# seongeunryu/lime-cikm25

Hardware: AMD Instinct MI355X
Metric: impressions scored/sec (higher is better)
Workload: dtype f32

## Files before the change

include/lime_hip.h:

```cpp
#ifndef LIME_HIP_H
#define LIME_HIP_H

#include <stdint.h>

#ifdef __cplusplus
extern "C" {
#endif

#define LIME_ABI_VERSION 14

typedef enum {
    LIME_OK = 0,
    LIME_ERR_BAD_ARG = -1,
    LIME_ERR_UNSUPPORTED = -2,
    LIME_ERR_LAUNCH = -3,
    LIME_NOT_APPLICABLE = 1
} lime_status;

int lime_abi_version(void);
const char* lime_last_error_string(void);
int64_t lime_device_cus(void);

enum { LIME_ACT_NONE = 0, LIME_ACT_RELU = 1, LIME_ACT_TANH = 2, LIME_ACT_SIGMOID = 3,
       LIME_ACT_RELU_GRAD = 4  };
// ... 97 lines not shown

int64_t lime_ffn_pack_sp_size(int32_t F, int32_t which);
int lime_ffn_pack_sp(const float* w1, int64_t ldw1, const float* w2, int64_t ldw2, int32_t E, int32_t F, uint16_t* w1p, uint16_t* w2p,
                     void* stream);

typedef struct {
    const float* attn;    int64_t lda;
    const uint16_t* wp;
    const float* bias;
    const float* res;     int64_t ldr;
    const int32_t* res_ids;
    const float* res_pe;  int64_t ldr_pe;
    int32_t res_period;
    float ln_eps;
    const float* ln_gamma; const float* ln_beta;
    float* out;           int64_t ldo;
    int32_t M, E;
    const int32_t* m_dev;
} lime_oproj_sp_args;

int lime_encoder_oproj_sp(const lime_oproj_sp_args* args, void* stream);

int64_t lime_oproj_pack_sp_size(void);
int lime_oproj_pack_sp(const float* w, int64_t ldw, int32_t E, uint16_t* wp, void* stream);

typedef struct {
    const uint16_t* attn; int64_t lda;
    const uint16_t* w0p;
    const float* add_rows; int64_t ld_add; int32_t add_period;
    int32_t res_kind;
    const uint16_t* res;  int64_t ldr;  int64_t res_rows;
    const int32_t* res_ids;
    const float* ln1_gamma; const float* ln1_beta; float ln1_eps;
    int32_t pool32;
    const uint16_t* w1p;  const uint16_t* w2p;  const float* b2;
    const float* ln2_gamma; const float* ln2_beta; float ln2_eps;
    int32_t M, E, F;
    void* out;            int64_t ldo;
    const int32_t* m_dev;
} lime_encoder_block_bf16_args;

int lime_encoder_block_bf16(const lime_encoder_block_bf16_args* args, void* stream);

int64_t lime_oproj_pack_bf16_size(void);
int lime_oproj_pack_bf16(const float* w, int64_t ldw, int32_t E, uint16_t* wp, void* stream);

typedef struct {
    const uint16_t* a;   int64_t lda;  int64_t a_rows;  const int32_t* a_ids;
    const uint16_t* wp;
    const float* add_rows; int64_t ld_add; int32_t add_period;
    int32_t M, N, K;
    int32_t reserved;
    const int32_t* c_ids;
    uint16_t* out;       int64_t ldo;  int64_t out_rows;
    const int32_t* m_dev;
} lime_inproj_bf16_args;

int lime_inproj_bf16(const lime_inproj_bf16_args* args, void* stream);
int64_t lime_inproj_pack_bf16_size(int32_t N);
int lime_inproj_pack_bf16(const float* w, int64_t ldw, int32_t N, int32_t K, uint16_t* wp, void* stream);

int32_t lime_ffn_bf16_model_columns(void);

int lime_to_bf16(const float* src, int64_t lds, int64_t rows, int32_t cols, uint16_t* dst, int64_t ldd, int64_t rows_out,
                 int32_t cols_out, void* stream);

int lime_mean_pool_bf16(const uint16_t* x, int64_t ldx, float* out, int64_t ldo, int32_t n_seq, int32_t S, int32_t dim,
                        void* stream);

int lime_embed_pe_f32(const int32_t* ids, const float* table, int64_t ld_table, const float* pe, int64_t ld_pe,
                      int32_t period, float* out, int64_t ldo, int64_t rows, int32_t dim, void* stream);

int lime_compact_sequences(const int32_t* ids, int32_t n_seq, int32_t S, int32_t pad_base, int32_t* seq_inv, int32_t* ids_c,
                           int32_t* row_map, int32_t* tok_ids, int32_t* tok_rows, int32_t* counts, int32_t* work, void* stream);

int lime_fill_pad_rows_f32(const int32_t* ids, const float* src, int64_t lds, float* dst, int64_t ldd, int64_t rows, int32_t S, int32_t cols,
                           void* stream);
int64_t lime_compact_sequences_workspace(int32_t n_seq);

int lime_compact_batch(const int32_t* ids_t, int32_t T, int32_t pad_base_t, int32_t* seq_inv_t, int32_t* ids_c_t, int32_t* row_map_t,
                       int32_t* tok_ids_t, int32_t* tok_rows_t, int32_t* counts_t, const int32_t* ids_b, int32_t L, int32_t pad_base_b,
                       int32_t* seq_inv_b, int32_t* ids_c_b, int32_t* row_map_b, int32_t* tok_ids_b, int32_t* tok_rows_b, int32_t* counts_b,
                       int32_t n, const int32_t* cat, const int32_t* sub, const float* fresh, const float* life, int32_t count_mult,
                       int32_t* news_src, int32_t* news_inv, int32_t* title_row, int32_t* body_row, int32_t* cat_c, int32_t* sub_c,
                       float* fresh_c, float* life_c, int32_t* news_counts, int32_t* work, void* stream);
int64_t lime_compact_batch_workspace(int32_t n);

int lime_news_xin_f32(const float* title_blocks, int64_t ld_t, int32_t nblk_t, const float* body_blocks, int64_t ld_b, int32_t nblk_b,
                      const int32_t* title_row, const int32_t* body_row, const int32_t* n_news, float* xin, int64_t ldx, int32_t cap,
                      int32_t dim, void* stream);

enum { LIME_ATTN_FORM_PLAIN = 0, LIME_ATTN_FORM_COUNT = 1, LIME_ATTN_FORM_LSE = 2, LIME_ATTN_FORM_ROWS = 3, LIME_ATTN_FORM_VOCAB = 4,
       LIME_ATTN_FORM_DROPOUT = 5 };
typedef struct {
    const float* q;
    const float* k;
    const float* v;
    int64_t ld_qkv;
    const float* pos_rows;
    const int32_t* row_map;
    const uint8_t* key_mask;
    const int32_t* n_seq_dev;
    float* lse;
    float* out;
    int64_t ldo;
    float* workspace;
    int64_t workspace_floats;
    uint64_t dropout_seed;
    float dropout_p;
    uint32_t dropout_site;
    int32_t n_seq, S, n_head, head_dim, head_stride;
    float scale;
    int32_t form;
    int32_t reserved;
} lime_token_attention_args;

int lime_token_attention_f32(const lime_token_attention_args* args, void* stream);

enum { LIME_ATTN_NONE = 0, LIME_ATTN_SP = 1, LIME_ATTN_SP_LONG = 2, LIME_ATTN_SP_VOCAB = 3, LIME_ATTN_MFMA = 4, LIME_ATTN_WIDE = 5,
       LIME_ATTN_DROPOUT = 6, LIME_ATTN_DROPOUT_LONG = 7 };
enum { LIME_ATTN_STATS_NONE = 0, LIME_ATTN_STATS_FP32 = 1, LIME_ATTN_STATS_SPLIT = 2 };
typedef struct {
    int32_t family;
    int32_t stats_pass;
    int32_t n_launches;
    int32_t reserved;
    char name[2][64];
} lime_token_attention_plan;

int lime_token_attention_plan_f32(const lime_token_attention_args* args, lime_token_attention_plan* out);

int lime_token_attention_rows_bf16(const uint16_t* q, const uint16_t* k, const uint16_t* v, int64_t ld_qkv, const int32_t* row_map,
                                   const int32_t* n_seq_dev, uint16_t* out, int64_t ldo, int32_t n_seq, int32_t S, int32_t n_head,
                                   int32_t head_dim, float scale, int32_t out_cols, void* stream);

int lime_token_attention_bf16(const uint16_t* q, const uint16_t* k, const uint16_t* v, int64_t ld_qkv, uint16_t* out,
                              int64_t ldo, int32_t n_seq, int32_t S, int32_t n_head, int32_t head_dim, float scale,
                              int32_t out_cols, void* stream);

int lime_pad_heads_f32(const float* src, int64_t lds, float* dst, int64_t ldd, int32_t n_blk, int32_t head_dim,
                       int32_t head_stride, int32_t cols, void* stream);

int lime_mean_pool_f32(const float* x, int64_t ldx, float* out, int64_t ldo, int32_t n_seq, int32_t S, int32_t dim,
                       void* stream);
int lime_mean_pool_count_f32(const float* x, int64_t ldx, float* out, int64_t ldo, int32_t n_seq, int32_t S, int32_t dim,
                             const int32_t* n_seq_dev, void* stream);

int lime_bucketize_f32(const float* x, int32_t* out, int64_t n, void* stream);
int lime_bucketize_cuts_f32(const float* x, const float* cuts, int32_t n_cuts, int32_t* out, int64_t n, void* stream);

int lime_topic_rep_f32(const int32_t* cat, const int32_t* sub, const float* cat_table, const float* sub_table,
                       int32_t dc, int32_t ds, const float* w, const float* bias, int32_t dout, float* out, int64_t ldo,
                       float* emb_out, int64_t ld_emb, int64_t rows, void* stream);

int lime_intent_fuse_f32(const float* intents, const float* att_hidden, const float* affine2_t, const float* affine2_b,
                         float* content, int64_t ldc, int64_t M, int32_t k, int32_t D, int32_t A, void* stream);
int lime_intent_fuse_count_f32(const float* intents, const float* att_hidden, const float* affine2_t, const float* affine2_b,
                               float* content, int64_t ldc, int64_t M, int32_t k, int32_t D, int32_t A, const int32_t* m_dev, void* stream);

int lime_additive_pool_f32(const float* hidden, int64_t ldh, const float* affine2, int32_t A, const float* x, int64_t ldx,
                           int32_t D, const uint8_t* mask, float* out, int64_t ldo, int32_t n_seq, int32_t S, void* stream);
int lime_additive_pool_count_f32(const float* hidden, int64_t ldh, const float* affine2, int32_t A, const float* x, int64_t ldx, int32_t D,
                                 const uint8_t* mask, const int32_t* n_seq_dev, float* out, int64_t ldo, int32_t n_seq, int32_t S, void* stream);

int lime_cand_attn_weights_f32(const float* qp, const float* kp, const uint8_t* mask, float* agg, int32_t B, int32_t N,
                               int32_t H, int32_t D, int32_t n_head, void* stream);
int64_t lime_cand_attn_weights_workspace(int32_t B, int32_t N, int32_t H, int32_t n_head);
int lime_cand_attn_weights_ws_f32(const float* qp, const float* kp, const uint8_t* mask, float* agg, int32_t B, int32_t N, int32_t H,
                                  int32_t D, int32_t n_head, float* workspace, int64_t workspace_floats, void* stream);
int lime_cand_attn_weights_shared_f32(const float* qp, const float* kp, const uint8_t* mask, float* agg, int32_t B, int32_t N, int32_t H,
                                      int32_t D, int32_t n_head, int32_t hist_div, float* workspace, int64_t workspace_floats, void* stream);

int lime_gate_ln_f32(const float* y, const float* x, const float* scale, const float* bias, const float* gamma,
                     const float* beta, float eps, float* out, int64_t rows, int32_t D, void* stream);

int lime_gate_ln_sage_f32(const float* y, const float* x, const float* scale, const float* bias, const float* gamma, const float* beta,
                          float eps, float* out, const float* node_const, float* mean_out, int64_t groups, int32_t H, int32_t D,
                          int32_t row_div, int32_t n_src, void* stream);

int lime_sage_mean_f32(const float* hist, const float* user_nodes, float* out, int32_t B, int32_t H, int32_t n_user,
                       int32_t n_src, int32_t D, void* stream);

int lime_interest_match_f32(const float* kp, const float* qp, const float* g, const float* cand, const float* remaining,
                            float* user_rep, float* logits, int32_t B, int32_t N, int32_t H, int32_t A, int32_t D,
                            float scale, float alpha_s, float beta_s, int32_t use_weight, int32_t use_penalty,
                            void* stream);

int lime_lifetime_score_f32(const float* user, const float* news, const float* remaining, float* logits, int64_t rows,
                            int32_t D, float alpha_s, float beta_s, int32_t use_weight, int32_t use_penalty, void* stream);

int lime_row_scale_f32(const float* x, const float* scale, float* out, int64_t rows, int32_t D, void* stream);

int lime_mhsa_live_ids(const int32_t* ids, const uint8_t* mask, int32_t n_seq, int32_t T, int32_t* ids_eff, void* stream);
int lime_mhsa_compact_mask(int32_t* ids_c, const int32_t* seq_src, const uint8_t* mask, int32_t n_compact_slots, int32_t T,
                           uint8_t* mask_c, void* stream);

int lime_fuse_rows_f32(const float* a, int64_t lda, const float* b, int64_t ldb, const float* gate, int64_t ldg, float* out, int64_t ldo,
                       int64_t rows, int32_t cols, void* stream);

int lime_gather_rows_f32(const int32_t* idx, const float* table, int64_t ld_table, float* out, int64_t ldo, int64_t rows,
                         int32_t dim, void* stream);

#define LIME_MAX_COPIES 32
typedef struct {
    const void* src;
    void* dst;
    int64_t bytes;
} lime_copy_desc;
int lime_multi_copy(const lime_copy_desc* descs, int32_t n, void* stream);

#define LIME_MAX_GATHERS 16
typedef struct {
    const void* table;  int64_t table_stride;
    void* out;          int64_t out_stride;
    int32_t row_bytes;  int32_t reserved;
} lime_gather_desc;
int lime_gather_rows_multi(const int32_t* idx, int64_t n_rows, const lime_gather_desc* descs, int32_t n, void* stream);


int64_t lime_linear_wgrad_workspace(int32_t M, int32_t N, int32_t K);
int lime_linear_wgrad_f32(const float* dy, int64_t ldy, const float* x, int64_t ldx, float* dw, int64_t lddw, float* db,
                          int32_t M, int32_t N, int32_t K, int32_t accumulate, float* workspace, int64_t workspace_floats,
                          void* stream);

int64_t lime_colsum_workspace(int32_t M, int32_t N);
int lime_colsum_f32(const float* x, int64_t ldx, int32_t M, int32_t N, float* out, int32_t accumulate, float* workspace,
                    int64_t workspace_floats, void* stream);

int64_t lime_layernorm_bwd_workspace(int32_t M, int32_t E);
int lime_layernorm_bwd_f32(const float* dy, int64_t lddy, int32_t dy_div, float dy_scale, const float* y, int64_t ldy,
                           const float* gamma, const float* beta, const float* rstd, float* dz, int64_t lddz, int32_t M,
                           int32_t E, float* dgamma, float* dbeta, float* dzsum, int32_t accumulate, float* workspace,
                           int64_t workspace_floats, void* stream);
int lime_layernorm_bwd_dropout_f32(const float* dy, int64_t lddy, int32_t dy_div, float dy_scale, const float* y, int64_t ldy,
                                   const float* gamma, const float* beta, const float* rstd, float* dz, int64_t lddz, int32_t M, int32_t E,
                                   float* dgamma, float* dbeta, float* dzsum, int32_t accumulate, float* workspace,
                                   int64_t workspace_floats, float* dz_drop, int64_t lddd, float dropout_p, uint64_t seed, uint32_t site,
                                   void* stream);

int lime_relu_bwd_f32(float* dh, int64_t lddh, const float* h, int64_t ldh, int64_t rows, int32_t cols, float scale, void* stream);

int64_t lime_token_attention_bwd_workspace(int32_t n_seq, int32_t S, int32_t n_head);
int64_t lime_token_attention_stats_workspace(int32_t n_seq, int32_t S, int32_t n_head);
int64_t lime_token_attention_bwd_workspace_wide(int32_t n_seq, int32_t S, int32_t n_head, int32_t head_dim);
enum { LIME_BWD_ATTN_ENTRY_PLAIN = 0, LIME_BWD_ATTN_ENTRY_LSE = 1 };
typedef struct {
    const float* q;
    const float* k;
    const float* v;
    int64_t ld_qkv;
    const float* out;
    int64_t ld_out;
    const float* lse;
    const float* dout;
    int64_t ldo;
    float* dq;
    float* dk;
    float* dv;
    int64_t ld_dqkv;
    float* workspace;
    int64_t workspace_floats;
    const uint8_t* key_mask;
    uint64_t dropout_seed;
    float dropout_p;
    uint32_t dropout_site;
    int32_t n_seq, S, n_head, head_dim, head_stride;
    float scale;
    int32_t entry;
    int32_t reserved;
} lime_token_attention_bwd_args;

int lime_token_attention_bwd_f32(const lime_token_attention_bwd_args* args, void* stream);

enum { LIME_BWD_ATTN_NONE = 0, LIME_BWD_ATTN_ONE_PASS = 1, LIME_BWD_ATTN_SP = 2, LIME_BWD_ATTN_LONG = 3, LIME_BWD_ATTN_LONG_SP = 4,
       LIME_BWD_ATTN_WIDE = 5 };
enum { LIME_BWD_ATTN_PASS_NONE = 0, LIME_BWD_ATTN_PASS_STATS_FP32 = 1, LIME_BWD_ATTN_PASS_STATS_SPLIT = 2, LIME_BWD_ATTN_PASS_DELTA = 3 };
typedef struct {
    int32_t family;
    int32_t stats_pass;
    int32_t n_launches;
    int32_t reserved;
    char name[3][64];
} lime_token_attention_bwd_plan;

int lime_token_attention_bwd_plan_f32(const lime_token_attention_bwd_args* args, lime_token_attention_bwd_plan* out);

int lime_additive_pool_bwd_f32(const float* hidden, int64_t ldh, const float* affine2, int32_t A, const float* x, int64_t ldx, int32_t D,
                               const uint8_t* mask, const float* dout, int64_t ldo, float* dhidden, int64_t lddh, float* dx, int64_t lddx,
                               float* da2_part, int32_t n_seq, int32_t S, void* stream);


int lime_dropout_f32(const float* src, int64_t lds, float* dst, int64_t ldd, int64_t rows, int32_t cols, float p, uint64_t seed,
                     uint32_t site, void* stream);
int lime_dropout2_f32(const float* src, int64_t lds, float* dst, int64_t ldd, int64_t rows, int32_t cols, float p, uint64_t seed,
                      uint32_t site1, uint32_t site2, void* stream);

int lime_embed_pe_dropout_f32(const int32_t* ids, const float* table, int64_t ld_table, const float* pe, int64_t ld_pe,
                              int32_t period, float* out, int64_t ldo, int64_t rows, int32_t dim, float p, uint64_t seed,
                              uint32_t site_emb, uint32_t site_pe, void* stream);

int lime_dropout_add_layernorm_f32(const float* t, int64_t ldt, const float* res, int64_t ldr, const float* gamma, const float* beta,
                                   float eps, float* y, int64_t ldy, float* rstd, int64_t M, int32_t E, float p, uint64_t seed,
                                   uint32_t site, void* stream);

int lime_embed_bwd_f32(const int32_t* ids, const float* dx, int64_t lddx, float* dtable, int64_t ld_table, int64_t rows,
                       int32_t dim, int32_t hot_id, void* stream);
// ... 222 lines not shown
```

lime_cikm25_amd/csrc/compact.hip:

```cpp
#include "common.h"

namespace {

__device__ __forceinline__ void count_seq(const int* __restrict__ ids, int s, int S, int* __restrict__ live_cnt) {
    const int lane = threadIdx.x & 63;
    int c = 0;
    for (int t = lane; t < S; t += 64) c += ids[(long)s * S + t] != 0;
#pragma unroll
    for (int o = 32; o > 0; o >>= 1) c += __shfl_xor(c, o);
    if (lane == 0) live_cnt[s] = c;
}

__global__ __launch_bounds__(256) void seq_count_kernel(const int* __restrict__ ids, int n_seq, int S, int* __restrict__ live_cnt) {
    const int s = blockIdx.x * 4 + (threadIdx.x >> 6);
    if (s >= n_seq) return;
    count_seq(ids, s, S, live_cnt);
}

__global__ __launch_bounds__(1024) void seq_scan_kernel(const int* __restrict__ live_cnt, int n_seq, int S, int* __restrict__ seq_src,
                                                        int* __restrict__ seq_inv, int* __restrict__ tok_off, int* __restrict__ counts) {
    __shared__ int part_seq[1024], part_tok[1024];
    const int tid = threadIdx.x;
    const int per = (n_seq + 1023) / 1024;
    const int lo = tid * per, hi = min(n_seq, lo + per);
    int ns = 0, nt = 0;
    for (int s = lo; s < hi; ++s) {
        const int c = live_cnt[s];
        ns += c > 0;
        nt += c;
    }
    part_seq[tid] = ns;
    part_tok[tid] = nt;
    __syncthreads();
    for (int o = 1; o < 1024; o <<= 1) {
        int a = 0, b = 0;
        if (tid >= o) { a = part_seq[tid - o]; b = part_tok[tid - o]; }
        __syncthreads();
        part_seq[tid] += a;
        part_tok[tid] += b;
        __syncthreads();
    }
    const int n_live = part_seq[1023], n_tok = part_tok[1023];
    int ps = part_seq[tid] - ns, pt = part_tok[tid] - nt;
    for (int s = lo; s < hi; ++s) {
        const int c = live_cnt[s];
        if (c > 0) {
            seq_src[ps] = s;
            seq_inv[s] = ps;
            tok_off[ps] = pt;
            ++ps;
            pt += c;
        } else {
            seq_inv[s] = n_live;
        }
    }
    for (int i = n_live + 1 + tid; i <= n_seq; i += 1024) seq_src[i] = -1;
    if (tid == 0) {
        seq_src[n_live] = -1;
        tok_off[n_live] = n_tok;
        counts[0] = n_live + 1;
        counts[1] = (n_live + 1) * S;
        counts[2] = n_tok;
        counts[3] = n_live;
        counts[4] = n_tok + S;
    }
}

__device__ __forceinline__ void emit_seq(const int cs, const int* __restrict__ ids, int S, const int* __restrict__ seq_src,
                                         const int* __restrict__ tok_off, const int* __restrict__ counts, int pad_base,
                                         int* __restrict__ ids_c, int* __restrict__ row_map, int* __restrict__ tok_ids,
                                         int* __restrict__ tok_rows) {
    const int lane = threadIdx.x & 63;
    const int n_c = counts[0];
    if (cs >= n_c) return;
    const int src = seq_src[cs];
    int base = tok_off[cs];
    for (int t0 = 0; t0 < S; t0 += 64) {
        const int t = t0 + lane;
        int id = 0;
        if (t < S && src >= 0) id = ids[(long)src * S + t];
        const bool live = id != 0;
        const unsigned long long m = __ballot(live);
        if (t < S) {
            const int row = cs * S + t;
            ids_c[row] = id;
            row_map[row] = live ? row : pad_base + t;
            if (cs == n_c - 1) {
                tok_ids[base + t] = 0;
                tok_rows[base + t] = pad_base + t;
            }
            if (live) {
                const int k = base + __popcll(m & ((1ull << lane) - 1ull));
                tok_ids[k] = id;
                tok_rows[k] = row;
            }
        }
        base += __popcll(m);
    }
}

__global__ __launch_bounds__(256) void seq_emit_kernel(const int* __restrict__ ids, int n_seq, int S, const int* __restrict__ seq_src,
                                                       const int* __restrict__ tok_off, const int* __restrict__ counts, int pad_base,
                                                       int* __restrict__ ids_c, int* __restrict__ row_map, int* __restrict__ tok_ids,
                                                       int* __restrict__ tok_rows) {
    emit_seq(blockIdx.x * 4 + (threadIdx.x >> 6), ids, S, seq_src, tok_off, counts, pad_base, ids_c, row_map, tok_ids, tok_rows);
}

struct SeqSide {
    const int* ids; int S, pad_base;
    int *live_cnt, *seq_src, *tok_off;
    int *seq_inv, *ids_c, *row_map, *tok_ids, *tok_rows, *counts;
};
struct NewsSide {
    const int *cat, *sub, *fresh, *life;
    int *news_src, *news_inv, *title_row, *body_row, *cat_c, *sub_c, *fresh_c, *life_c, *counts;
    int count_mult;
};

__global__ __launch_bounds__(256) void batch_count_kernel(const SeqSide t, const SeqSide b, int n) {
    const int w = blockIdx.x * 4 + (threadIdx.x >> 6);
    if (w >= 2 * n) return;
    if (w < n) count_seq(t.ids, w, t.S, t.live_cnt);
    else count_seq(b.ids, w - n, b.S, b.live_cnt);
}

__device__ __forceinline__ void scan_side_write(const SeqSide& d, int n, int lo, int hi, int ps, int pt, int n_live, int n_tok) {
    const int tid = threadIdx.x;
    for (int s = lo; s < hi; ++s) {
        const int c = d.live_cnt[s];
        if (c > 0) {
            d.seq_src[ps] = s;
            d.seq_inv[s] = ps;
            d.tok_off[ps] = pt;
            ++ps;
            pt += c;
        } else {
            d.seq_inv[s] = n_live;
        }
    }
    for (int i = n_live + 1 + tid; i <= n; i += 1024) d.seq_src[i] = -1;
    if (tid == 0) {
        d.seq_src[n_live] = -1;
        d.tok_off[n_live] = n_tok;
        d.counts[0] = n_live + 1;
        d.counts[1] = (n_live + 1) * d.S;
        d.counts[2] = n_tok;
        d.counts[3] = n_live;
        d.counts[4] = n_tok + d.S;
    }
}

__global__ __launch_bounds__(1024) void batch_scan_kernel(const SeqSide t, const SeqSide b, const NewsSide w, int n) {
    __shared__ int part[5][1024];
    const int tid = threadIdx.x;
    const int per = (n + 1023) / 1024;
    const int lo = min(n, tid * per), hi = min(n, lo + per);
    int first = 0x7FFFFFFF;
    for (int s = hi - 1; s >= lo; --s)
        if (t.live_cnt[s] == 0 && b.live_cnt[s] == 0) first = s;
    part[0][tid] = first;
    __syncthreads();
    for (int o = 512; o > 0; o >>= 1) {
        if (tid < o) part[0][tid] = min(part[0][tid], part[0][tid + o]);
        __syncthreads();
    }
    first = part[0][0];
    __syncthreads();
    const bool has_pad = first != 0x7FFFFFFF;
    int kc = 0, ks = 0, kf = 0, kl = 0;
    if (has_pad) { kc = w.cat[first]; ks = w.sub[first]; kf = w.fresh[first]; kl = w.life[first]; }
    auto repeats = [&](int s) {
        return has_pad && t.live_cnt[s] == 0 && b.live_cnt[s] == 0 && w.cat[s] == kc && w.sub[s] == ks && w.fresh[s] == kf && w.life[s] == kl;
    };
    int v[5] = {0, 0, 0, 0, 0};
    for (int s = lo; s < hi; ++s) {
        const int ct = t.live_cnt[s], cb = b.live_cnt[s];
        v[0] += ct > 0; v[1] += ct;
        v[2] += cb > 0; v[3] += cb;
        v[4] += !repeats(s);
    }
#pragma unroll
    for (int i = 0; i < 5; ++i) part[i][tid] = v[i];
    __syncthreads();
    for (int o = 1; o < 1024; o <<= 1) {
        int a[5] = {0, 0, 0, 0, 0};
        if (tid >= o) {
#pragma unroll
            for (int i = 0; i < 5; ++i) a[i] = part[i][tid - o];
        }
        __syncthreads();
#pragma unroll
        for (int i = 0; i < 5; ++i) part[i][tid] += a[i];
        __syncthreads();
    }
    scan_side_write(t, n, lo, hi, part[0][tid] - v[0], part[1][tid] - v[1], part[0][1023], part[1][1023]);
    scan_side_write(b, n, lo, hi, part[2][tid] - v[2], part[3][tid] - v[3], part[2][1023], part[3][1023]);
    const int n_live = part[4][1023];
    int pn = part[4][tid] - v[4];
    for (int s = lo; s < hi; ++s) {
        if (repeats(s)) {
            w.news_inv[s] = n_live;
        } else {
            w.news_src[pn] = s;
            w.news_inv[s] = pn;
            ++pn;
        }
    }
    for (int i = n_live + 1 + tid; i <= n; i += 1024) w.news_src[i] = -1;
    if (tid == 0) {
        const int n_news = n_live + (has_pad ? 1 : 0);
        w.news_src[n_live] = has_pad ? first : -1;
        w.counts[0] = n_news;
        w.counts[1] = w.count_mult * n_news;
        w.counts[2] = n_live;
        w.counts[3] = has_pad ? first : -1;
    }
}

__global__ __launch_bounds__(256) void batch_emit_kernel(const SeqSide t, const SeqSide b, const NewsSide w, int n, int seq_blocks) {
    const int blk = blockIdx.x;
    const int wave = threadIdx.x >> 6;
    if (blk < seq_blocks) {
        emit_seq(blk * 4 + wave, t.ids, t.S, t.seq_src, t.tok_off, t.counts, t.pad_base, t.ids_c, t.row_map, t.tok_ids, t.tok_rows);
        return;
    }
    if (blk < 2 * seq_blocks) {
        emit_seq((blk - seq_blocks) * 4 + wave, b.ids, b.S, b.seq_src, b.tok_off, b.counts, b.pad_base, b.ids_c, b.row_map, b.tok_ids, b.tok_rows);
        return;
    }
    const int j = (blk - 2 * seq_blocks) * 256 + threadIdx.x;
    if (j > n) return;
    const int src = j < w.counts[0] ? w.news_src[j] : -1;
    const bool on = src >= 0;
    w.title_row[j] = on ? t.seq_inv[src] : 0;
    w.body_row[j] = on ? b.seq_inv[src] : 0;
    w.cat_c[j] = on ? w.cat[src] : 0;
    w.sub_c[j] = on ? w.sub[src] : 0;
    w.fresh_c[j] = on ? w.fresh[src] : 0;
    w.life_c[j] = on ? w.life[src] : 0;
}

}

extern "C" int lime_compact_sequences(const int32_t* ids, int32_t n_seq, int32_t S, int32_t pad_base, int32_t* seq_inv, int32_t* ids_c,
                                      int32_t* row_map, int32_t* tok_ids, int32_t* tok_rows, int32_t* counts, int32_t* work, void* stream) {
    LIME_REQUIRE(ids && seq_inv && ids_c && row_map && tok_ids && tok_rows && counts && work, LIME_ERR_BAD_ARG, "lime_compact_sequences: NULL pointer");
    LIME_REQUIRE(n_seq > 0 && S > 0 && pad_base >= 0, LIME_ERR_BAD_ARG, "lime_compact_sequences: bad dims n_seq=%d S=%d pad_base=%d", n_seq, S, pad_base);
    LIME_REQUIRE((long)(n_seq + 1) * S + S < 0x7FFFFFFFL && (long)pad_base + S < 0x7FFFFFFFL, LIME_ERR_UNSUPPORTED, "lime_compact_sequences: too many rows");
    hipStream_t s = (hipStream_t)stream;
    int* live_cnt = work;
    int* seq_src = work + n_seq;
    int* tok_off = work + 2 * n_seq + 1;
    hipLaunchKernelGGL(seq_count_kernel, dim3((n_seq + 3) / 4), dim3(256), 0, s, ids, n_seq, S, live_cnt);
    hipLaunchKernelGGL(seq_scan_kernel, dim3(1), dim3(1024), 0, s, live_cnt, n_seq, S, seq_src, seq_inv, tok_off, counts);
    hipLaunchKernelGGL(seq_emit_kernel, dim3((n_seq + 1 + 3) / 4), dim3(256), 0, s, ids, n_seq, S, seq_src, tok_off, counts, pad_base, ids_c,
                       row_map, tok_ids, tok_rows);
    return lime_check_launch("lime_compact_sequences");
}

extern "C" int64_t lime_compact_sequences_workspace(int32_t n_seq) { return 3L * n_seq + 2; }

extern "C" int lime_compact_batch(const int32_t* ids_t, int32_t T, int32_t pad_base_t, int32_t* seq_inv_t, int32_t* ids_c_t, int32_t* row_map_t,
                                  int32_t* tok_ids_t, int32_t* tok_rows_t, int32_t* counts_t, const int32_t* ids_b, int32_t L, int32_t pad_base_b,
                                  int32_t* seq_inv_b, int32_t* ids_c_b, int32_t* row_map_b, int32_t* tok_ids_b, int32_t* tok_rows_b,
                                  int32_t* counts_b, int32_t n, const int32_t* cat, const int32_t* sub, const float* fresh, const float* life,
                                  int32_t count_mult, int32_t* news_src, int32_t* news_inv, int32_t* title_row, int32_t* body_row,
                                  int32_t* cat_c, int32_t* sub_c, float* fresh_c, float* life_c, int32_t* news_counts, int32_t* work,
                                  void* stream) {
    LIME_REQUIRE(ids_t && seq_inv_t && ids_c_t && row_map_t && tok_ids_t && tok_rows_t && counts_t && ids_b && seq_inv_b && ids_c_b &&
                     row_map_b && tok_ids_b && tok_rows_b && counts_b && work,
                 LIME_ERR_BAD_ARG, "lime_compact_batch: NULL pointer (sequence level)");
    LIME_REQUIRE(cat && sub && fresh && life && news_src && news_inv && title_row && body_row && cat_c && sub_c && fresh_c && life_c && news_counts,
                 LIME_ERR_BAD_ARG, "lime_compact_batch: NULL pointer (news level)");
    LIME_REQUIRE(n > 0 && T > 0 && L > 0 && pad_base_t >= 0 && pad_base_b >= 0 && count_mult >= 1, LIME_ERR_BAD_ARG,
                 "lime_compact_batch: bad dims n=%d T=%d L=%d pad_base=%d/%d count_mult=%d", n, T, L, pad_base_t, pad_base_b, count_mult);
    LIME_REQUIRE((long)(n + 1) * T + T < 0x7FFFFFFFL && (long)pad_base_t + T < 0x7FFFFFFFL && (long)(n + 1) * L + L < 0x7FFFFFFFL &&
                     (long)pad_base_b + L < 0x7FFFFFFFL && (long)count_mult * (n + 1) < 0x7FFFFFFFL,
                 LIME_ERR_UNSUPPORTED, "lime_compact_batch: too many rows");
    hipStream_t s = (hipStream_t)stream;
    int* const work_b = work + 3L * n + 2;
    const SeqSide t = {ids_t, T, pad_base_t, work, work + n, work + 2 * n + 1, seq_inv_t, ids_c_t, row_map_t, tok_ids_t, tok_rows_t, counts_t};
    const SeqSide b = {ids_b, L, pad_base_b, work_b, work_b + n, work_b + 2 * n + 1, seq_inv_b, ids_c_b, row_map_b, tok_ids_b, tok_rows_b, counts_b};
    const NewsSide w = {cat, sub, (const int*)fresh, (const int*)life, news_src, news_inv, title_row, body_row, cat_c, sub_c,
                        (int*)fresh_c, (int*)life_c, news_counts, count_mult};
    const int seq_blocks = (n + 1 + 3) / 4;
    hipLaunchKernelGGL(batch_count_kernel, dim3((unsigned)((2L * n + 3) / 4)), dim3(256), 0, s, t, b, n);
    hipLaunchKernelGGL(batch_scan_kernel, dim3(1), dim3(1024), 0, s, t, b, w, n);
    hipLaunchKernelGGL(batch_emit_kernel, dim3((unsigned)(2 * seq_blocks + (n + 1 + 255) / 256)), dim3(256), 0, s, t, b, w, n, seq_blocks);
    return lime_check_launch("lime_compact_batch");
}

extern "C" int64_t lime_compact_batch_workspace(int32_t n) { return 2 * (3L * n + 2); }
```

lime_cikm25_amd/csrc/news_tail_f32.hip:

```cpp
#include "common.h"

namespace {

__global__ __launch_bounds__(64) void topic_rep_kernel(const int* __restrict__ cat, const int* __restrict__ sub,
                                                        const float* __restrict__ cat_table, const float* __restrict__ sub_table,
                                                        int dc, int ds, const float* __restrict__ w, const float* __restrict__ bias,
                                                        int dout, float* __restrict__ out, long ldo, float* __restrict__ emb_out,
                                                        long ld_emb) {
    __shared__ float e[256];
    const long r = blockIdx.x;
    const int din = dc + ds;
    const float* crow = cat_table + (long)cat[r] * dc;
    const float* srow = sub_table + (long)sub[r] * ds;
    for (int i = threadIdx.x; i < din; i += 64) {
        const float v = (i < dc) ? crow[i] : srow[i - dc];
        e[i] = v;
        if (emb_out) emb_out[r * ld_emb + i] = v;
    }
    __syncthreads();
    if (out) {
        for (int o = threadIdx.x; o < dout; o += 64) {
            const float* wr = w + (long)o * din;
            float acc = 0.f;
            for (int i = 0; i < din; ++i) acc += wr[i] * e[i];
            out[r * ldo + o] = acc + (bias ? bias[o] : 0.f);
        }
    }
}

}

extern "C" int lime_topic_rep_f32(const int32_t* cat, const int32_t* sub, const float* cat_table, const float* sub_table,
                                  int32_t dc, int32_t ds, const float* w, const float* bias, int32_t dout, float* out,
                                  int64_t ldo, float* emb_out, int64_t ld_emb, int64_t rows, void* stream) {
    LIME_REQUIRE(cat && sub && cat_table && sub_table, LIME_ERR_BAD_ARG, "lime_topic_rep_f32: NULL pointer");
    LIME_REQUIRE(out || emb_out, LIME_ERR_BAD_ARG, "lime_topic_rep_f32: nothing to write");
    LIME_REQUIRE(!out || (w && dout > 0 && ldo >= dout), LIME_ERR_BAD_ARG, "lime_topic_rep_f32: out needs w, dout, ldo");
    LIME_REQUIRE(dc > 0 && ds > 0 && dc + ds <= 256, LIME_ERR_UNSUPPORTED, "lime_topic_rep_f32: dc + ds must be in (0, 256]");
    LIME_REQUIRE(!emb_out || ld_emb >= dc + ds, LIME_ERR_BAD_ARG, "lime_topic_rep_f32: ld_emb too small");
    if (rows <= 0) return rows == 0 ? LIME_OK : LIME_ERR_BAD_ARG;
    hipLaunchKernelGGL(topic_rep_kernel, dim3((unsigned)rows), dim3(64), 0, (hipStream_t)stream, cat, sub, cat_table, sub_table, dc,
                       ds, w, bias, dout, out, (long)ldo, emb_out, (long)ld_emb);
    return lime_check_launch("lime_topic_rep_f32");
}

namespace {

constexpr int MAX_INTENT = 8;

__global__ __launch_bounds__(256) void intent_fuse_kernel(const float* __restrict__ intents, const float* __restrict__ hidden,
                                                           const float* __restrict__ aff2_t, const float* __restrict__ aff2_b,
                                                           float* __restrict__ content, long ldc, long M, int k, int D, int A,
                                                           const int* __restrict__ m_dev) {
    extern __shared__ __attribute__((aligned(16))) float sm[];
    float* pooled = sm;
    float* red = sm + 2 * D;
    const long m = blockIdx.x;
    if (m_dev && m >= (long)*m_dev) return;
    for (int tb = 0; tb < 2; ++tb) {
        const float* aff2 = tb == 0 ? aff2_t : aff2_b;
        const float* hid = hidden + ((long)tb * M + m) * k * A;
        const float* itn = intents + ((long)tb * M + m) * k * D;
        float a[MAX_INTENT];
        float mx = -INFINITY;
        for (int kk = 0; kk < k; ++kk) {
            float part = 0.f;
            for (int j = threadIdx.x; j < A; j += 256) part += hid[kk * A + j] * aff2[j];
            a[kk] = block_sum(part, red);
            mx = fmaxf(mx, a[kk]);
        }
        float den = 0.f;
        for (int kk = 0; kk < k; ++kk) {
            a[kk] = expf(a[kk] - mx);
            den += a[kk];
        }
        const float inv = 1.0f / den;
        for (int d = threadIdx.x; d < D; d += 256) {
            float x = 0.f;
            for (int kk = 0; kk < k; ++kk) x += (a[kk] * inv) * itn[kk * D + d];
            pooled[tb * D + d] = x;
        }
    }
    __syncthreads();
    float dot = 0.f, n1 = 0.f, n2 = 0.f;
    for (int d = threadIdx.x; d < D; d += 256) {
        const float t = pooled[d], b = pooled[D + d];
        dot += t * b;
        n1 += t * t;
        n2 += b * b;
    }
    dot = block_sum(dot, red);
    n1 = block_sum(n1, red);
    n2 = block_sum(n2, red);
    const float cosv = dot / (fmaxf(sqrtf(n1), 1e-8f) * fmaxf(sqrtf(n2), 1e-8f));
    const float s = (cosv + 1.0f) * 0.5f;
    for (int d = threadIdx.x; d < D; d += 256) {
        content[m * ldc + d] = pooled[d];
        content[m * ldc + D + d] = s * pooled[D + d];
    }
}

}

static int intent_fuse(const float* intents, const float* att_hidden, const float* affine2_t, const float* affine2_b, float* content,
                       int64_t ldc, int64_t M, int32_t k, int32_t D, int32_t A, const int32_t* m_dev, void* stream) {
    LIME_REQUIRE(intents && att_hidden && affine2_t && affine2_b && content, LIME_ERR_BAD_ARG, "lime_intent_fuse_f32: NULL pointer");
    LIME_REQUIRE(M >= 0 && k > 0 && D > 0 && A > 0 && ldc >= 2 * (int64_t)D, LIME_ERR_BAD_ARG, "lime_intent_fuse_f32: bad dims");
    LIME_REQUIRE(k <= MAX_INTENT && D <= 4096, LIME_ERR_UNSUPPORTED, "lime_intent_fuse_f32: k <= 8 and D <= 4096 only");
    if (M == 0) return LIME_OK;
    const size_t lds = (size_t)(2 * D + 4) * sizeof(float);
    hipLaunchKernelGGL(intent_fuse_kernel, dim3((unsigned)M), dim3(256), lds, (hipStream_t)stream, intents, att_hidden, affine2_t,
                       affine2_b, content, (long)ldc, (long)M, k, D, A, m_dev);
    return lime_check_launch("lime_intent_fuse_f32");
}

extern "C" int lime_intent_fuse_f32(const float* intents, const float* att_hidden, const float* affine2_t,
                                    const float* affine2_b, float* content, int64_t ldc, int64_t M, int32_t k, int32_t D,
                                    int32_t A, void* stream) {
    return intent_fuse(intents, att_hidden, affine2_t, affine2_b, content, ldc, M, k, D, A, nullptr, stream);
}

extern "C" int lime_intent_fuse_count_f32(const float* intents, const float* att_hidden, const float* affine2_t, const float* affine2_b,
                                          float* content, int64_t ldc, int64_t M, int32_t k, int32_t D, int32_t A, const int32_t* m_dev,
                                          void* stream) {
    LIME_REQUIRE(m_dev, LIME_ERR_BAD_ARG, "lime_intent_fuse_count_f32: NULL count");
    return intent_fuse(intents, att_hidden, affine2_t, affine2_b, content, ldc, M, k, D, A, m_dev, stream);
}

namespace {

__global__ __launch_bounds__(256) void additive_pool_kernel(const float* __restrict__ hidden, long ldh,
                                                             const float* __restrict__ aff2, int A, const float* __restrict__ x,
                                                             long ldx, int D, const unsigned char* __restrict__ mask,
                                                             float* __restrict__ out, long ldo, int S, const int* __restrict__ n_seq_dev) {
    __shared__ float alpha[512];
    __shared__ float red[4];
    const long s = blockIdx.x;
    if (n_seq_dev != nullptr && (int)blockIdx.x >= *n_seq_dev) return;
    const int lane = threadIdx.x & 63, wave = threadIdx.x >> 6;
    for (int t = wave; t < S; t += 4) {
        const float* h = hidden + (s * S + t) * ldh;
        float part = 0.f;
        for (int j = lane; j < A; j += 64) part += h[j] * aff2[j];
        part = wave_sum(part);
        if (lane == 0) alpha[t] = (mask && mask[s * S + t] == 0) ? -1e9f : part;
    }
    __syncthreads();
    const float inv = block_softmax_terms(alpha, S, red);
    __syncthreads();
    for (int d = threadIdx.x; d < D; d += 256) {
        float acc = 0.f;
        for (int t = 0; t < S; ++t) acc += (alpha[t] * inv) * x[(s * S + t) * ldx + d];
        out[s * ldo + d] = acc;
    }
}

}

extern "C" int lime_additive_pool_count_f32(const float* hidden, int64_t ldh, const float* affine2, int32_t A, const float* x,
                                            int64_t ldx, int32_t D, const uint8_t* mask, const int32_t* n_seq_dev, float* out, int64_t ldo,
                                            int32_t n_seq, int32_t S, void* stream) {
    LIME_REQUIRE(hidden && affine2 && x && out, LIME_ERR_BAD_ARG, "lime_additive_pool_f32: NULL pointer");
    LIME_REQUIRE(n_seq >= 0 && S > 0 && A > 0 && D > 0 && ldh >= A && ldx >= D && ldo >= D, LIME_ERR_BAD_ARG,
                 "lime_additive_pool_f32: bad dims");
    LIME_REQUIRE(S <= 512, LIME_ERR_UNSUPPORTED, "lime_additive_pool_f32: S %d > 512", S);
    if (n_seq == 0) return LIME_OK;
    hipLaunchKernelGGL(additive_pool_kernel, dim3((unsigned)n_seq), dim3(256), 0, (hipStream_t)stream, hidden, (long)ldh, affine2, A,
                       x, (long)ldx, D, mask, out, (long)ldo, S, n_seq_dev);
    return lime_check_launch("lime_additive_pool_f32");
}

extern "C" int lime_additive_pool_f32(const float* hidden, int64_t ldh, const float* affine2, int32_t A, const float* x,
                                      int64_t ldx, int32_t D, const uint8_t* mask, float* out, int64_t ldo, int32_t n_seq,
                                      int32_t S, void* stream) {
    return lime_additive_pool_count_f32(hidden, ldh, affine2, A, x, ldx, D, mask, nullptr, out, ldo, n_seq, S, stream);
}
```

lime_cikm25_amd/model.py:

```python
import functools
import os

import torch
import torch.nn as nn

from . import newsEncoders, ops, serving, training, userEncoders
from .util import RemainingLifetimeWeighting

_USED = (1, 2, 3, 4, 6, 9, 10, 11, 15, 16, 17, 18, 20, 23, 24, 25)
_PAIRS = ((17, 3), (18, 4), (20, 6), (15, 1), (16, 2), (23, 9), (24, 10))
_USED_BODY_MASK = tuple(sorted(_USED + (7, 21)))
_PAIRS_BODY_MASK = _PAIRS + ((21, 7),)
_USED_TITLE_ENTITY = tuple(sorted(_USED + (5, 19)))
_PAIRS_TITLE_ENTITY = _PAIRS + ((19, 5),)


_USER_ENCODERS = ('CROWN', 'ATT', 'MHSA')
_CONTENT_ENCODERS = ('CROWN', 'CNN', 'NAML', 'MHSA', 'CNE', 'KCNN')
_PLAIN_NEWS_ENCODERS = ('CROWN', 'CNN', 'NAML', 'MHSA', 'KCNN')
_REFUSED_USER_ENCODERS = {
    'LSTUR': ' (it needs user_ID embeddings and a GRU)', 'GRU': ' (it needs a GRU over the history)',
    'PUE': ' (it needs user_ID embeddings)', 'CATT': ' (it pools the history per candidate)',
    'MINER': ' (poly attention with per-candidate pooling)', 'SUE': ' (it is not part of this port)',
    'FIM': ' (it needs the HDC news encoder and the FIM click predictor)',
}


_REFUSED_CLICK_PREDICTORS = {
    'sigmoid': ' (the reference\'s forward has no branch for it: model.py:179-186 leaves logits unset)',
    'FIM': ' (it needs the HDC news encoder and the FIM user encoder, model.py:108-110)',
}


INDEXED_MATCH = os.environ.get('LIME_INDEXED_MATCH', '1') != '0'
OCCURRENCE_MATCH = os.environ.get('LIME_OCCURRENCE_MATCH', '0') != '0'
SCHEDULE_MATCH = os.environ.get('LIME_SCHEDULE_MATCH', '1') != '0'


class Model(nn.Module):

    def __init__(self, config):
        super().__init__()
        self.config = config
        if config.news_encoder == 'LIME':
            if config.content_encoder not in _CONTENT_ENCODERS:
                raise NotImplementedError('content_encoder %r is a baseline outside the scoring path' % config.content_encoder)
            base_encoder = getattr(newsEncoders, config.content_encoder)(config)
            self.news_encoder = newsEncoders.LIME(config=config, base_news_encoder=base_encoder)
        elif config.news_encoder in _PLAIN_NEWS_ENCODERS:
            base_encoder = self.news_encoder = getattr(newsEncoders, config.news_encoder)(config)
        elif config.news_encoder == 'CNE':
            raise NotImplementedError('news_encoder \'CNE\' without LIME stays refused: its gates pair the news of an encoder call, so it '
                                      'has no per-news cache, and its 1,700-column representation is outside the refinement kernels -- '
                                      'use news_encoder=\'LIME\' with content_encoder=\'CNE\'')
        else:
            raise NotImplementedError('news_encoder %r: the MI355X path covers LIME (config.py:25) and the baselines %s' % (
                config.news_encoder, ', '.join(_PLAIN_NEWS_ENCODERS)))
        if config.user_encoder not in _USER_ENCODERS:
            raise NotImplementedError('user_encoder %r is outside the scoring path%s: the supported user encoders are %s' % (
                config.user_encoder, _REFUSED_USER_ENCODERS.get(config.user_encoder, ''), ', '.join(sorted(_USER_ENCODERS))))
        if config.user_encoder == 'CROWN' and config.news_encoder not in ('LIME', 'CROWN'):
            raise NotImplementedError('user_encoder \'CROWN\' needs the news encoder\'s category_affine over the (category, subCategory) '
                                      'pair (userEncoders.py:103-105): news_encoder %r has %s -- pair it with ATT or MHSA, or put it under LIME'
                                      % (config.news_encoder, 'a category_affine of another shape' if hasattr(self.news_encoder, 'category_affine')
                                         else 'no category_affine'))
        self.user_encoder = getattr(userEncoders, config.user_encoder)(self.news_encoder, config)
        self.plain = config.news_encoder != 'LIME'
        self.model_name = (f"{config.news_encoder}-{config.user_encoder}" if self.plain else
                           f"{config.news_encoder}-{config.content_encoder}-{config.user_encoder}")
        self.news_embedding_dim = self.news_encoder.news_embedding_dim
        self.dropout = nn.Dropout(p=config.dropout_rate)
        self.use_user_embedding = False
        self.click_predictor = config.click_predictor
        if self.click_predictor == 'mlp':
            self.mlp = nn.Linear(in_features=self.news_embedding_dim * 2, out_features=self.news_embedding_dim // 2, bias=True)
            self.out = nn.Linear(in_features=self.news_embedding_dim // 2, out_features=1, bias=True)
        elif self.click_predictor != 'dot_product':
            raise NotImplementedError('click_predictor %r stays refused%s: the supported click predictors are dot_product (config.py:109) '
                                      'and mlp' % (self.click_predictor, _REFUSED_CLICK_PREDICTORS.get(self.click_predictor, '')))
        self.remaining_lifetime_weighting = RemainingLifetimeWeighting(config)
        self._regular_offsets = {}
        self.use_graph = True
        self._graphs = {}
        self.reads_content_mask = bool(getattr(base_encoder, 'reads_content_mask', False))
        self.reads_title_entity = bool(getattr(base_encoder, 'reads_title_entity', False))
        self._used = _USED_BODY_MASK if self.reads_content_mask else _USED_TITLE_ENTITY if self.reads_title_entity else _USED
        self._pairs = _PAIRS_BODY_MASK if self.reads_content_mask else _PAIRS_TITLE_ENTITY if self.reads_title_entity else _PAIRS

    @property
    def content_encoder(self):
        return self.news_encoder if self.plain else self.news_encoder.base_news_encoder

    def _apply(self, fn, *args, **kwargs):
        self._graphs = {}
        self._regular_offsets = {}
        self._products_key = None
        return super()._apply(fn, *args, **kwargs)

    def weights_changed(self):
        ops.note_param_write()

    def _sync_weight_products(self):
        enc = self.content_encoder
        if hasattr(enc, 'products_key'):
            key = enc.products_key()
            if key != getattr(self, '_products_key', None):
                self._products_key = key
                self._graphs = {}

    def initialize(self):
        self.news_encoder.initialize()
        self.user_encoder.initialize()
        if self.click_predictor == 'mlp':
            nn.init.xavier_uniform_(self.mlp.weight, gain=nn.init.calculate_gain('relu'))
            nn.init.zeros_(self.mlp.bias)
        self.remaining_lifetime_weighting.initialize()

    def forward(self, user_ID, user_category, user_subCategory, user_title_text, user_title_mask, user_title_entity,
                user_content_text, user_content_mask, user_content_entity, user_freshness, user_user_topic_lifetime,
                user_history_mask, user_history_graph, user_history_category_mask, user_history_category_indices, news_category,
                news_subCategory, news_title_text, news_title_mask, news_title_entity, news_content_text, news_content_mask,
                news_content_entity, news_freshness, news_user_topic_lifetime, remaining_lifetime):
        args = (user_ID, user_category, user_subCategory, user_title_text, user_title_mask, user_title_entity,
                user_content_text, user_content_mask, user_content_entity, user_freshness, user_user_topic_lifetime,
                user_history_mask, user_history_graph, user_history_category_mask, user_history_category_indices, news_category,
                news_subCategory, news_title_text, news_title_mask, news_title_entity, news_content_text, news_content_mask,
                news_content_entity, news_freshness, news_user_topic_lifetime, remaining_lifetime)
        self.news_encoder.auxiliary_loss = None
        if self.training and (torch.is_grad_enabled() or self.news_encoder.training or self.user_encoder.training):
            return training.forward_train(self, user_category, user_subCategory, user_title_text, user_title_mask,
                                          user_content_text, user_freshness, user_user_topic_lifetime, user_history_mask,
                                          news_category, news_subCategory, news_title_text, news_title_mask, news_content_text,
                                          news_freshness, news_user_topic_lifetime, remaining_lifetime,
                                          user_content_mask=user_content_mask if self.reads_content_mask else None,
                                          news_content_mask=news_content_mask if self.reads_content_mask else None,
                                          user_title_entity=user_title_entity if self.reads_title_entity else None,
                                          news_title_entity=news_title_entity if self.reads_title_entity else None)
        if (self.use_graph and ops.PROFILE is None and user_category.is_cuda
                and not torch.cuda.is_current_stream_capturing()):
            self._sync_weight_products()
            return self._forward_graphed(args)
        return self._forward_impl(*args)

    def _forward_graphed(self, args):
        _USED = self._used
        used = [args[i] for i in _USED]
        key = (self.training,) + tuple((tuple(t.shape), t.dtype) for t in used)
        entry = self._graphs.get(key)
        if entry is None:
            static = list(args)
            for i, t in zip(_USED, self._packed_like(args, _USED, self._pairs)):
                static[i] = t
            ops.multi_copy([(static[i], args[i]) for i in _USED])
            with torch.no_grad():
                self._forward_impl(*static)
            torch.cuda.synchronize()
            graph = torch.cuda.CUDAGraph()
            with torch.cuda.graph(graph):
                out = self._forward_impl(*static)
            entry = (graph, [static[i] for i in _USED], out)
            self._graphs[key] = entry
            enc = self.content_encoder
            if hasattr(enc, 'products_key'):
                self._products_key = enc.products_key()
        graph, static_used, out = entry
        keep = ops.multi_copy(list(zip(static_used, used)))
        graph.replay()
        del keep
        return out.clone()

    @staticmethod
    def _packed_like(args, _USED=_USED, _PAIRS=_PAIRS):
        order = list(_USED)
        for n_i, u_i in _PAIRS:
            order.remove(u_i)
            order.insert(order.index(n_i) + 1, u_i)
        offs, total = {}, 0
        for i in order:
            t = args[i]
            adjacent = any(i == u and args[n].dtype == t.dtype for n, u in _PAIRS)
            if not adjacent:
                total = (total + 255) // 256 * 256
            offs[i] = total
            total += t.numel() * t.element_size()
        buf = torch.empty(total + 256, dtype=torch.uint8, device=args[_USED[0]].device)
        base = (-buf.data_ptr()) % 256
        out = []
        for i in _USED:
            t = args[i]
            nbytes = t.numel() * t.element_size()
            out.append(buf[base + offs[i]:base + offs[i] + nbytes].view(t.dtype).view(t.shape))
        return out

    @torch.no_grad()
    def score_impressions(self, user_category, user_subCategory, user_title_text, user_title_mask, user_content_text,
                          user_freshness, user_user_topic_lifetime, user_history_mask, news_category, news_subCategory,
                          news_title_text, news_title_mask, news_content_text, news_freshness, news_user_topic_lifetime,
                          remaining_lifetime, n_src=None, rows_per_pass=16384, user_content_mask=None, news_content_mask=None,
                          user_title_entity=None, news_title_entity=None):
        B, K = news_category.shape
        H = user_category.shape[1]
        if self.reads_content_mask:
            if user_content_mask is None or news_content_mask is None:
                raise TypeError('the CNE content encoder reads the body masks (user_content_mask, news_content_mask): pass them -- '
                                'a body mask is never guessed from the ids')
            if self.training:
                raise RuntimeError('score_impressions is the eval-mode function: call model.eval() first')
            rows = lambda t: t.reshape((B * K,) + tuple(t.shape[2:]))
            rep = lambda t: t.repeat_interleave(K, dim=0)
            if news_user_topic_lifetime.dim() == 1:
                news_user_topic_lifetime = news_user_topic_lifetime.unsqueeze(1).expand(B, K)
            if news_freshness.dim() == 1:
                news_freshness = news_freshness.unsqueeze(1).expand(B, K)
            logits = self._forward_impl(None, rep(user_category), rep(user_subCategory), rep(user_title_text), rep(user_title_mask), None,
                                        rep(user_content_text), rep(user_content_mask), None, rep(user_freshness),
                                        rep(user_user_topic_lifetime), rep(user_history_mask), None, None, None, rows(news_category),
                                        rows(news_subCategory), rows(news_title_text), rows(news_title_mask), None,
                                        rows(news_content_text), rows(news_content_mask), None, rows(news_freshness.contiguous()),
                                        rows(news_user_topic_lifetime.contiguous()), rows(remaining_lifetime))
            return logits.view(B, K)
        ne, ue = self.news_encoder, self.user_encoder
        if self.reads_title_entity and (user_title_entity is None or news_title_entity is None):
            raise TypeError('the KCNN content encoder reads the title entity ids (user_title_entity, news_title_entity): pass them -- '
                            'the ids are never guessed')
        if not self.reads_title_entity:
            user_title_entity = news_title_entity = None
        if news_user_topic_lifetime.dim() == 1:
            news_user_topic_lifetime = news_user_topic_lifetime.unsqueeze(1).expand(B, K)
        if news_freshness.dim() == 1:
            news_freshness = news_freshness.unsqueeze(1).expand(B, K)
        cand, hist = ne.encode_many([
            (news_title_text, news_title_mask, news_content_text, news_category, news_subCategory, news_freshness.contiguous(),
             news_user_topic_lifetime.contiguous(), None, news_title_entity),
            (user_title_text, user_title_mask, user_content_text, user_category, user_subCategory, user_freshness,
             user_user_topic_lifetime, None, user_title_entity)])
        rows = B * K
        if n_src is None and hasattr(ue, 'user_node_embedding'):
            n_src = min(rows, H + ue.user_node_embedding.shape[0])
        out = torch.empty((B, K), dtype=torch.float32, device=cand.device)
        per = max(1, rows_per_pass // K)
        n_pass = (B + per - 1) // per
        per = (B + n_pass - 1) // n_pass
        rl = remaining_lifetime.float()
        gate_y = ue.gate_projection(hist)
        for b0 in range(0, B, per):
            b1 = min(B, b0 + per)
            n = (b1 - b0) * K
            logits = self._row_logits(hist[b0:b1], news_category[b0:b1].reshape(n, 1), news_subCategory[b0:b1].reshape(n, 1),
                                      user_category[b0:b1], user_subCategory[b0:b1], user_history_mask[b0:b1],
                                      cand[b0:b1].reshape(n, 1, -1), rl[b0:b1].reshape(n, 1), n_src=n_src, hist_div=K,
                                      gate_y=None if gate_y is None else gate_y[b0 * H:b1 * H])
            out[b0:b1] = logits.view(b1 - b0, K)
        return out

    @torch.no_grad()
    def build_news_cache(self, device_corpus, rows_per_pass=8192):
        c = device_corpus
        if self.reads_content_mask:
            return torch.empty((c.news_title_text.shape[0], 0), dtype=torch.float32, device=c.news_title_text.device)
        return self.news_encoder.build_content_cache(c.news_title_text, c.news_title_mask, c.news_abstract_text, c.news_category,
                                                     c.news_subCategory, rows_per_pass=rows_per_pass,
                                                     title_entity=c.news_title_entity if self.reads_title_entity else None)

    def build_recurrence_cache(self, device_corpus, news_per_pass=None):
        if self.config.content_encoder != 'CNE':
            raise ValueError('content_encoder %r has no recurrence cache (it is the CNE content encoder\'s): use build_news_cache'
                             % self.config.content_encoder)
        c = device_corpus
        return self.news_encoder.base_news_encoder.build_recurrence_cache(c.news_title_text, c.news_title_mask, c.news_abstract_text,
                                                                          c.news_abstract_mask, news_per_pass=news_per_pass)

    @torch.no_grad()
    def score_behaviors(self, behaviors, rows, news_cache, n_src=None, recurrence_cache=None, rows_per_forward=None):
        if recurrence_cache is not None:
            if self.config.content_encoder != 'CNE':
                raise ValueError('content_encoder %r does not read a recurrence cache (it is the CNE content encoder\'s)'
                                 % self.config.content_encoder)
            return self._score_from_recurrence(behaviors, rows, recurrence_cache, n_src, rows_per_forward)
        b = behaviors
        dev = news_cache.device
        rows = torch.as_tensor(rows, device=dev).long().reshape(-1)
        R, H = rows.numel(), b.hist_index.shape[1]
        ne, ue, c = self.news_encoder, self.user_encoder, b.corpus
        hist_idx, cand_idx = b.hist_index[rows], b.cand_index[rows]
        flat_h, flat_c = hist_idx.reshape(-1).long(), cand_idx.reshape(-1).long()
        remaining = self._remaining_lifetime(b, rows, cand_idx)
        if self.reads_content_mask:
            return self._forward_impl(*b.assemble(rows), remaining.view(R)).view(R)
        hist = ne.encode_cached(news_cache, hist_idx, b.user_freshness[rows], b.user_lifetime[rows]).view(R, H, -1)
        cand = ne.encode_cached(news_cache, cand_idx, b.cand_freshness[rows], b.cand_lifetime[rows]).view(R, 1, -1)
        if n_src is None and hasattr(ue, 'user_node_embedding'):
            n_src = min(R, H + ue.user_node_embedding.shape[0])
        logits = self._row_logits(hist, c.news_category[flat_c].view(R, 1), c.news_subCategory[flat_c].view(R, 1),
                                  c.news_category[flat_h].view(R, H), c.news_subCategory[flat_h].view(R, H), b.hist_mask[rows],
                                  cand, remaining.view(R, 1), n_src=n_src)
        return logits.view(R)

    def _remaining_lifetime(self, behaviors, rows, cand_idx):
        b = behaviors
        return self._lifetime_rule(b.cand_freshness[rows], lambda: b.cand_lifetime[rows],
                                   lambda: b.corpus.news_category[cand_idx.reshape(-1).long()])

    def _lifetime_rule(self, freshness, lifetime, category):
        lt = getattr(self.config, 'lifetime_type', 'user_topic')
        if lt == 'fixed':
            return self.config.fixed_lifetime - freshness
        if lt == 'topic_wise':
            cmap = torch.as_tensor(self.config.category_lifetime_map, dtype=torch.float32, device=freshness.device)
            return cmap[category().long()].view_as(freshness) - freshness
        if lt == 'user_topic':
            return lifetime() - freshness
        raise ValueError('Invalid lifetime_type')

    _NO_CONTENT_CACHE = ('content_encoder \'CNE\' has no per-news content cache (its gates read the partner news of the encoder call, '
                         'build_news_cache): score_pool / recommend cannot serve it -- score the pairs with score_behaviors')

    def grouped_by(self):
# ... 218 lines not shown
```

lime_cikm25_amd/newsEncoders.py:

```python
import collections
import math
import os
import types

import torch
import torch.nn as nn
from torch.nn import TransformerEncoder, TransformerEncoderLayer

from . import ops
from .layers import Attention, Conv1D, Conv2D_Pool, LinearHolder, LSTMHolder, MultiHeadAttention, ScaledDotProduct_CandidateAttention

MAX_TOKENS_PER_PASS = 4 * 1024 * 1024

DEDUP = os.environ.get('LIME_DENSE_TOKENS', '0') != '1'
NEWS_DEDUP = os.environ.get('LIME_NEWS_DEDUP', '1') != '0'


def _no_train_dropout(module, p):
    if module.training and p > 0:
        raise NotImplementedError('encode_flat() is the fused scoring kernel chain (eval-mode children, or dropout_rate = 0): with '
                                  'training-mode dropout active call the module (forward) or Model.forward, which take the '
                                  'differentiable path of lime_cikm25_amd.training')


# ... 80 lines not shown
            mid = (lo + hi) // 2
            if int(f([mid])[0]) >= k:
                hi = mid
            else:
                lo = mid
        win = list(range(max(one, hi - 64), min(top, hi + 64) + 1))
        b = f(win)
        if not bool(((b >= k) == (torch.tensor(win) >= hi)).all()):
            raise ValueError('the bucket rule is not monotone around its cut point %d (num_buckets = %d)' % (k, num_buckets))
        cuts.append(hi)
    return torch.from_numpy(np.array(cuts, dtype=np.uint32).view(np.float32).copy())


class FreshnessEncoder(nn.Module):

    def __init__(self, config, base_news_encoder):
        super().__init__()
        embedding_dim = config.freshness_embedding_dim
        hidden_dim = base_news_encoder.news_embedding_dim
        self.num_buckets = config.num_buckets
        self._cuts = None if self.num_buckets == 10 else bucket_cut_points(self.num_buckets)
        self.freshness_embedding = nn.Embedding(self.num_buckets, embedding_dim)
        self.lifetime_embedding = nn.Embedding(self.num_buckets, embedding_dim)
        self.dense = nn.Linear(embedding_dim * 2, hidden_dim)
        self.activation = nn.Tanh()

    def bucketize(self, x):
        return self.buckets(x.float()).long()

    def cuts_on(self, device):
        if self._cuts is not None and self._cuts.device != device:
            self._cuts = self._cuts.to(device)
        return self._cuts

    def buckets(self, x):
        return ops.bucketize(x, self.cuts_on(x.device))

    def encode_flat(self, freshness, lifetime, out):
        M = freshness.numel()
        E = self.freshness_embedding.embedding_dim
        fb = self.buckets(freshness)
        lb = self.buckets(lifetime)
        cat = torch.empty((M, 2 * E), dtype=torch.float32, device=out.device)
        ops.gather_rows(fb, self.freshness_embedding.weight, cat[:, :E])
        ops.gather_rows(lb, self.lifetime_embedding.weight, cat[:, E:])
        return ops.linear(cat, self.dense.weight, self.dense.bias, act='tanh', out=out)

    def forward(self, news_freshness, news_user_topic_lifetime):
        if news_freshness.dim() == 1:
            news_freshness = news_freshness.unsqueeze(1)
        if news_user_topic_lifetime.dim() == 1:
            news_user_topic_lifetime = news_user_topic_lifetime.unsqueeze(1)
        if news_freshness.shape != news_user_topic_lifetime.shape:
            news_user_topic_lifetime = news_user_topic_lifetime.expand_as(news_freshness)
        B, n = news_freshness.shape
        out = torch.empty((B * n, self.dense.out_features), dtype=torch.float32, device=news_freshness.device)
        self.encode_flat(news_freshness.float().contiguous().view(-1), news_user_topic_lifetime.float().contiguous().view(-1), out)
        return out.view(B, n, -1)


class LIME(nn.Module):

    def __init__(self, config, base_news_encoder):
        super().__init__()
        self.final_dim = config.lime_output_dim
        self.category_embedding = nn.Embedding(config.category_num, config.category_embedding_dim)
        self.category_embedding.weight.requires_grad = False
        self.subCategory_embedding = nn.Embedding(config.subCategory_num, config.subCategory_embedding_dim)
        self.subCategory_embedding.weight.requires_grad = False
        self.category_affine = nn.Linear(config.category_embedding_dim + config.subCategory_embedding_dim,
                                         config.category_embedding_dim)
        self.base_news_encoder = base_news_encoder
        self.freshness_encoder = FreshnessEncoder(config, base_news_encoder)
        self.fusion_method = config.fusion_method
        self.auxiliary_loss = getattr(base_news_encoder, 'auxiliary_loss', None)
        content_dim = self.base_news_encoder.news_embedding_dim
        freshness_dim = content_dim
        if self.fusion_method == 'concat':
            self.output_dim = content_dim + freshness_dim
            if self.final_dim:
                self.project = nn.Linear(self.output_dim, self.final_dim)
                self.output_dim = self.final_dim
            else:
                self.project = nn.Identity()
        elif self.fusion_method == 'add':
            self.output_dim = content_dim
            self.project = nn.Identity()
        elif self.fusion_method == 'gated':
            self.gate = nn.Linear(content_dim + freshness_dim, content_dim)
            self.output_dim = content_dim
            self.project = nn.Identity()
        else:
            raise ValueError('Unknown fusion method: %s' % self.fusion_method)
        self.news_embedding_dim = self.output_dim

    def initialize(self):
        if hasattr(self.base_news_encoder, 'initialize'):
            self.base_news_encoder.initialize()
        nn.init.xavier_uniform_(self.freshness_encoder.dense.weight)
        nn.init.zeros_(self.freshness_encoder.dense.bias)
        nn.init.uniform_(self.category_embedding.weight, -0.1, 0.1)
        nn.init.uniform_(self.subCategory_embedding.weight, -0.1, 0.1)
        nn.init.xavier_uniform_(self.category_affine.weight)
        nn.init.zeros_(self.category_affine.bias)

    def _base_encode(self, title_text, title_mask, content_text, category, subCategory, out, content_mask, pair_groups=None,
                     title_entity=None, recurrence=None):
        enc = self.base_news_encoder
        if recurrence is not None:
            return enc.encode_cached_flat(recurrence[0], recurrence[1], title_mask, content_mask, category, subCategory, out, pair_groups)
        if getattr(enc, 'reads_title_entity', False):
            return enc.encode_flat(title_text, title_mask, content_text, category, subCategory, out, title_entity=title_entity)
        if getattr(enc, 'reads_content_mask', False):
            return enc.encode_flat(title_text, title_mask, content_text, category, subCategory, out, content_mask, pair_groups)
        return enc.encode_flat(title_text, title_mask, content_text, category, subCategory, out)

    def encode_flat(self, title_text, title_mask, content_text, category, subCategory, freshness, lifetime, content_mask=None,
                    pair_groups=None, title_entity=None, recurrence=None):
        M = category.shape[0]
        dev = category.device
        cdim = self.base_news_encoder.news_embedding_dim
        main = torch.cuda.current_stream()
        side = _side_stream(dev)
        if self.fusion_method in ('add', 'gated'):
            fused = torch.empty((M, 2 * cdim), dtype=torch.float32, device=dev)
            side.wait_stream(main)
            with torch.cuda.stream(side):
                self.freshness_encoder.encode_flat(freshness, lifetime, fused[:, cdim:])
            self._base_encode(title_text, title_mask, content_text, category, subCategory, fused[:, :cdim], content_mask, pair_groups,
                              title_entity, recurrence)
            main.wait_stream(side)
            gate = ops.linear(fused, self.gate.weight, self.gate.bias, act='sigmoid') if self.fusion_method == 'gated' else None
            return ops.fuse_rows(fused[:, :cdim], fused[:, cdim:], gate)
        if isinstance(self.project, nn.Identity):
            fused = torch.empty((M, 2 * cdim), dtype=torch.float32, device=dev)
            side.wait_stream(main)
            with torch.cuda.stream(side):
                self.freshness_encoder.encode_flat(freshness, lifetime, fused[:, cdim:])
            self._base_encode(title_text, title_mask, content_text, category, subCategory, fused[:, :cdim], content_mask, pair_groups,
                              title_entity, recurrence)
            main.wait_stream(side)
            return fused
        fe = self.freshness_encoder
        nb = fe.num_buckets
        enc = self.base_news_encoder
        if (NEWS_DEDUP and recurrence is None and title_text is not None and hasattr(enc, 'news_dedup_applicable') and
                enc.news_dedup_applicable(title_text, content_text)):
            side3 = _side_stream(dev, 3)
            side3.wait_stream(main)
            with torch.cuda.stream(side3):
                news = ops.compact_batch(title_text, content_text, category, subCategory, freshness.contiguous(), lifetime.contiguous(),
                                         count_mult=enc.intent_num)
            nw = news[2]
            side.wait_stream(main)
            with torch.cuda.stream(side):
                side.wait_event(nw.ready)
                pair = torch.add(fe.buckets(nw.life_c), fe.buckets(nw.fresh_c), alpha=nb)
                table, _ = self.occurrence_tables()
            content = torch.empty((M + 1, cdim), dtype=torch.float32, device=dev)
            enc.encode_flat(title_text, title_mask, content_text, category, subCategory, content, news=news)
            main.wait_stream(side)
            rep_c = ops.linear(content, self.project.weight[:, :cdim], None, res=table, res_ids=pair, m_dev=nw.n_news)
            return ops.gather_rows(nw.news_inv, rep_c, torch.empty((M, rep_c.shape[1]), dtype=torch.float32, device=dev))
        side.wait_stream(main)
        with torch.cuda.stream(side):
            pair = torch.add(fe.buckets(lifetime), fe.buckets(freshness), alpha=nb)
            table, _ = self.occurrence_tables()
        content = torch.empty((M, cdim), dtype=torch.float32, device=dev)
        self._base_encode(title_text, title_mask, content_text, category, subCategory, content, content_mask, pair_groups, title_entity,
                          recurrence)
        main.wait_stream(side)
        return ops.linear(content, self.project.weight[:, :cdim], None, res=table, res_ids=pair)

    def occurrence_tables(self):
        fe = self.freshness_encoder
        E, nb = fe.freshness_embedding.embedding_dim, fe.num_buckets
        cdim = self.base_news_encoder.news_embedding_dim
        t_f, t_l = ops.linear_group([dict(a=fe.freshness_embedding.weight, w=fe.dense.weight[:, :E], bias=None),
                                     dict(a=fe.lifetime_embedding.weight, w=fe.dense.weight[:, E:], bias=fe.dense.bias)])
        fresh = torch.tanh(t_f.unsqueeze(1) + t_l.unsqueeze(0)).view(nb * nb, -1)
        if self.fusion_method == 'gated':
            return fresh, ops.linear(fresh, self.gate.weight[:, cdim:], self.gate.bias)
        if self.fusion_method == 'concat' and not isinstance(self.project, nn.Identity):
            return ops.linear(fresh, self.project.weight[:, cdim:], self.project.bias), None
        return fresh, None

    def occurrence_ids(self, freshness, lifetime):
        fe = self.freshness_encoder
        fr, lt = freshness.float().reshape(-1).contiguous(), lifetime.float().reshape(-1).contiguous()
        return torch.add(fe.buckets(lt), fe.buckets(fr), alpha=fe.num_buckets)

    def occurrence_ids_schedule(self, freshness, lifetime):
        fe = self.freshness_encoder
        S = freshness.shape[0]
        fr, lt = freshness.float().reshape(-1).contiguous(), lifetime.float().reshape(-1).contiguous()
        return torch.add(fe.buckets(lt).unsqueeze(0), fe.buckets(fr).view(S, -1), alpha=fe.num_buckets)

    def build_content_cache(self, title_text, title_mask, content_text, category, subCategory, rows_per_pass=8192, title_entity=None):
        n = title_text.shape[0]
        reads_entity = getattr(self.base_news_encoder, 'reads_title_entity', False)
        if reads_entity and title_entity is None:
            raise TypeError('the KCNN content encoder reads the title entity ids: pass title_entity -- the ids are never guessed')
        cdim = self.base_news_encoder.news_embedding_dim
        dev = title_text.device
        ident = isinstance(self.project, nn.Identity)
        gated = self.fusion_method == 'gated'
        cache = torch.empty((n, 2 * cdim if gated else cdim if ident else self.project.out_features), dtype=torch.float32, device=dev)
        direct = gated or ident
        for r0 in range(0, n, rows_per_pass):
            r1 = min(n, r0 + rows_per_pass)
            content = cache[r0:r1, :cdim] if direct else torch.empty((r1 - r0, cdim), dtype=torch.float32, device=dev)
            kw = dict(title_entity=_i32(title_entity[r0:r1]).contiguous()) if reads_entity else {}
            self.base_news_encoder.encode_flat(_i32(title_text[r0:r1]).contiguous(), title_mask[r0:r1].contiguous(),
                                               _i32(content_text[r0:r1]).contiguous(), _i32(category[r0:r1]).contiguous(),
                                               _i32(subCategory[r0:r1]).contiguous(), content, **kw)
            if gated:
                ops.linear(content, self.gate.weight[:, :cdim], None, out=cache[r0:r1, cdim:])
            elif not ident:
                ops.linear(content, self.project.weight[:, :cdim], None, out=cache[r0:r1])
        return cache

    def encode_cached(self, cache, news_index, freshness, lifetime, fused=None):
        cdim = self.base_news_encoder.news_embedding_dim
        R = news_index.numel()
        idx = _i32(news_index.reshape(-1)).contiguous()
        fr, lt = freshness.float().reshape(-1).contiguous(), lifetime.float().reshape(-1).contiguous()
        ident = isinstance(self.project, nn.Identity)
        if self.fusion_method != 'concat' or (not ident and (ops.FUSED_OCCURRENCE if fused is None else fused)):
            T, Q = self.occurrence_tables()
            A, P = (cache[:, :cdim], cache[:, cdim:]) if self.fusion_method == 'gated' else (cache, None)
            return ops.cached_occurrence(self.fusion_method, idx, fr, lt, A, T, P, Q, cuts=self.freshness_encoder.cuts_on(cache.device))
        fresh = torch.empty((R, cdim), dtype=torch.float32, device=cache.device)
        self.freshness_encoder.encode_flat(fr, lt, fresh)
        if ident:
            return torch.cat([cache[idx.long()], fresh], dim=1)
        return ops.linear(fresh, self.project.weight[:, cdim:], self.project.bias, res=cache, res_ids=idx)

    def encode_many(self, groups):
        shapes, flat, cmasks, ents = [], [[] for _ in range(7)], [], []
        for group in groups:
            tt, tm, ct, cat, sub, fr, lt = group[:7]
            if len(group) > 7 and group[7] is not None:
                cmasks.append(group[7].reshape(tt.shape[0] * tt.shape[1], -1))
            if len(group) > 8 and group[8] is not None:
                ents.append(_i32(group[8]).reshape(tt.shape[0] * tt.shape[1], -1))
            B, n = tt.shape[0], tt.shape[1]
            shapes.append((B, n))
            if fr.dim() == 1:
                fr = fr.unsqueeze(1)
            if lt.dim() == 1:
                lt = lt.unsqueeze(1)
            if lt.shape != fr.shape:
                lt = lt.expand_as(fr)
            for dst, t in zip(flat, (_i32(tt).reshape(B * n, -1), tm.reshape(B * n, -1), _i32(ct).reshape(B * n, -1),
                                     _i32(cat).reshape(-1), _i32(sub).reshape(-1), fr.float().reshape(-1), lt.float().reshape(-1))):
                dst.append(t)
        cat_all = [t[0].contiguous() if len(t) == 1 else _cat_rows(t) for t in flat]
        if cmasks and len(cmasks) != len(groups):
            raise ValueError('encode_many: the body mask must be given for every group or for none')
        cmask = None if not cmasks else (cmasks[0].contiguous() if len(cmasks) == 1 else _cat_rows(cmasks))
        if ents and len(ents) != len(groups):
            raise ValueError('encode_many: the title entity ids must be given for every group or for none')
        if getattr(self.base_news_encoder, 'reads_title_entity', False) and not ents:
            raise TypeError('the KCNN content encoder reads the title entity ids: every group needs them -- the ids are never guessed')
        ent = None if not ents else (ents[0].contiguous() if len(ents) == 1 else _cat_rows(ents))
        out = self.encode_flat(*cat_all, content_mask=cmask, pair_groups=[B * n for B, n in shapes] if cmask is not None else None,
                               title_entity=ent)
        res, r0 = [], 0
        for (B, n) in shapes:
            res.append(out[r0:r0 + B * n].view(B, n, -1))
            r0 += B * n
        return res

    def forward(self, title_text, title_mask, title_entity, content_text, content_mask, content_entity, category, subCategory,
                user_embedding, news_freshness=None, news_user_topic_lifetime=None):
        from . import training
        if training.wants_train_path(self, getattr(self.base_news_encoder, 'dropout_rate', 0.0)):
            B, n = title_text.shape[0], title_text.shape[1]
            fr, lt = news_freshness, news_user_topic_lifetime
            fr = fr.unsqueeze(1) if fr.dim() == 1 else fr
            lt = lt.unsqueeze(1) if lt.dim() == 1 else lt
            lt = lt.expand_as(fr) if lt.shape != fr.shape else lt
            rep = training.news_flat(self, *_flat_inputs(title_text, title_mask, content_text, category, subCategory),
                                     fr.float().reshape(-1).contiguous(), lt.float().reshape(-1).contiguous(),
                                     content_mask=None if content_mask is None else content_mask.reshape(B * n, -1).contiguous(),
                                     pair_groups=[B * n], title_entity=self._entity_rows(title_entity, B * n))
            return rep.view(B, n, -1)
        reads_entity = getattr(self.base_news_encoder, 'reads_title_entity', False)
        return self.encode_many([(title_text, title_mask, content_text, category, subCategory, news_freshness,
                                  news_user_topic_lifetime, content_mask, title_entity if reads_entity else None)])[0]

    def _entity_rows(self, title_entity, rows):
        if not getattr(self.base_news_encoder, 'reads_title_entity', False) or title_entity is None:
            return None
        return _i32(title_entity).reshape(rows, -1).contiguous()


class NewsEncoder(nn.Module):

    def __init__(self, config):
        super().__init__()
        self.word_embedding_dim = config.word_embedding_dim
        self.category_num = config.category_num
        self.word_embedding = nn.Embedding(num_embeddings=config.vocabulary_size, embedding_dim=self.word_embedding_dim)
        self.category_embedding = nn.Embedding(num_embeddings=config.category_num, embedding_dim=config.category_embedding_dim)
        self.category_embedding.weight.requires_grad = False
        self.subCategory_embedding = nn.Embedding(num_embeddings=config.subCategory_num,
                                                  embedding_dim=config.subCategory_embedding_dim)
        self.subCategory_embedding.weight.requires_grad = False
        self.dropout_rate = config.dropout_rate
        self.dropout = nn.Dropout(p=config.dropout_rate, inplace=True)
        self.dropout_ = nn.Dropout(p=config.dropout_rate, inplace=False)
        self.auxiliary_loss = None
        self.affine = nn.Linear(config.word_embedding_dim, config.word_embedding_dim, bias=True)

    reads_content_mask = False
    reads_title_entity = False

    def initialize(self):
        nn.init.uniform_(self.category_embedding.weight, -0.1, 0.1)
        nn.init.uniform_(self.subCategory_embedding.weight, -0.1, 0.1)
        nn.init.zeros_(self.subCategory_embedding.weight[0])
        nn.init.xavier_uniform_(self.affine.weight)
        nn.init.zeros_(self.affine.bias)

    def forward(self, title_text, title_mask, title_entity, content_text, content_mask, content_entity, category, subCategory,
                user_embedding, news_freshness=None, news_user_topic_lifetime=None):
# ... 259 lines not shown


def oproj_sp_rule(on, split_on, M, E, has_bias, aligned):
    return bool(on and split_on and 0 < E <= 304 and E % 4 == 0 and has_bias and aligned and M >= 4096 and (M + 127) // 128 >= 160)


def _oproj_sp_applicable(sa, attn, res):
    M, E = attn.shape
    ok16 = lambda t: t is None or (t.stride(1) == 1 and t.stride(0) % 4 == 0 and t.data_ptr() % 16 == 0)
    return oproj_sp_rule(SP_OPROJ, ops.split_gemm_on(), M, E, sa.out_proj.bias is not None,
                         ok16(attn) and ok16(res['res']) and ok16(res.get('res_pe')))


_IDENT = {}


def _identity_rows(n, device):
    return _grown(_IDENT, n, device, 4096, lambda size: torch.arange(size, dtype=torch.int32, device=device))


def compact_run(prep, table, pe, transformer, nhead, pooled_out, blocks_only=False):
    cmp, w_in, pew, qkv, prod = prep
    rows = _Rows(cmp.n_seq + 1, cmp.S, cmp.tok_ids, cmp.ids_c, w_in, pew, qkv, c_ids=cmp.tok_rows, m_tok=cmp.n_live_tokens,
                 m_rows=cmp.n_rows, n_seq_dev=cmp.n_compact, row_map=cmp.row_map, seq_inv=cmp.seq_inv, ew=prod.get('ew'),
                 ffn=prod.get('ffn'), oproj=prod.get('oproj'))
    return _encode_layers(rows, table, pe, transformer, nhead, pooled_out, blocks_only)


def compact_applicable(ids, table, transformer, nhead):
    M, S = ids.shape
    E = table.shape[1]
    return (DEDUP and len(transformer.layers) >= 1 and transformer.norm is None and E % nhead == 0 and E // nhead <= 32 and
            E % 4 == 0 and S % 32 == 0 and (S // 32 <= 4 or S // 32 in (8, 16)) and (M + 1) * S >= 4096 and
            ids.dtype == torch.int32 and ids.is_contiguous())


FUSED_FFN = os.environ.get('LIME_BF16_FUSED_FFN', '1') != '0'
FUSED_BLOCK = FUSED_FFN and os.environ.get('LIME_BF16_FUSED_BLOCK', '1') != '0'


def _inproj_applicable(N, K):
    return FUSED_FFN and N % 320 == 0 and K <= 320 and K % 8 == 0


def _ffn_fused_applicable(layer, E, EP):
    return (FUSED_FFN and EP == ops.ffn_model_columns() and EP - 15 <= E < EP and layer.linear1.out_features % 128 == 0 and
            layer.linear1.bias is not None and layer.linear2.bias is not None)


def _pack_layer_bf16(layer, first, pe, S, EP, nhead):
    sa = layer.self_attn
    E = pe.shape[1]
    hd = E // nhead
    padv = lambda v: torch.cat([v, v.new_zeros(EP - E)])
    p = types.SimpleNamespace(inproj=_inproj_applicable(3 * nhead * 32, EP), ffn=_ffn_fused_applicable(layer, E, EP))
    p.block = FUSED_BLOCK and p.ffn and E % 4 == 0
    w_in = ops.pad_heads(sa.in_proj_weight, 3 * nhead, hd, 32)
    b_in = ops.pad_heads(sa.in_proj_bias, 3 * nhead, hd, 32)
    p.w_in = ops.inproj_pack_bf16(w_in, EP) if p.inproj else ops.to_bf16(w_in, cols_out=EP)
    p.in_rows = ops.linear(pe[:S], w_in, b_in) if first else b_in.view(1, -1) if p.inproj else b_in
    if p.ffn:
        p.w1p, p.w2p = ops.ffn_pack_bf16(layer.linear1.weight, layer.linear1.bias, layer.linear2.weight)
    else:
        p.w1, p.w2 = ops.to_bf16(layer.linear1.weight, cols_out=EP), ops.to_bf16(layer.linear2.weight, rows_out=EP)
        p.b2, p.ln2 = padv(layer.linear2.bias), (padv(layer.norm2.weight), padv(layer.norm2.bias))
    if p.block:
        p.w0p = ops.oproj_pack_bf16(sa.out_proj.weight)
        p.add_rows = pe[:S] + sa.out_proj.bias if first else sa.out_proj.bias.view(1, E)
    else:
        p.w_o, p.b_o = ops.to_bf16(sa.out_proj.weight, rows_out=EP, cols_out=EP), padv(sa.out_proj.bias)
        p.ln1 = (padv(layer.norm1.weight), padv(layer.norm1.bias))
        p.pe_p = torch.cat([pe[:S], pe.new_zeros(S, EP - E)], dim=1) if first else None
    return p


def _encode_layers_bf16(ids, cmp, table_bf16, pe, transformer, nhead, pooled_out, shared=None):
    M, S = ids.shape
    EP = table_bf16.shape[1]
    E = pe.shape[1]
    hd = E // nhead
    if hd > 32 or S % 32 != 0:
        raise NotImplementedError('the bf16 encoder path needs head_dim <= 32 and S a multiple of 32 (got %d, %d)' % (hd, S))
    if transformer.norm is not None:
        raise NotImplementedError('a final encoder norm is not used by the reference (newsEncoders.py:245,247)')
    W = nhead * 32
    scale = 1.0 / math.sqrt(hd)
    shared = {} if shared is None else shared
    if cmp is None:
        n_seq, a_ids, res_ids, c_ids, n_seq_dev, rows = M, ids.reshape(-1), ids.reshape(-1), None, None, {}
    else:
        n_seq, a_ids, res_ids, c_ids, n_seq_dev, rows = M + 1, cmp.tok_ids, cmp.ids_c, cmp.tok_rows, cmp.n_compact, dict(m_dev=cmp.n_rows)
    cap = n_seq * S
    x = None
    for li, layer in enumerate(transformer.layers):
        if li not in shared:
            shared[li] = _pack_layer_bf16(layer, li == 0, pe, S, EP, nhead)
        p = shared[li]
        qkv = torch.empty((cap if cmp is None else cap + S, 3 * W), dtype=torch.bfloat16, device=ids.device)
        if li > 0 and p.inproj:
            ops.inproj_bf16(x, p.w_in, p.in_rows, 3 * W, qkv)
        elif li > 0:
            ops.linear_bf16(x, p.w_in, p.in_rows, n_alg=3 * E, k_alg=E, out=qkv)
        elif p.inproj:
            ops.inproj_bf16(table_bf16, p.w_in, p.in_rows, 3 * W, qkv, a_ids=a_ids, c_ids=c_ids,
                            m_dev=None if cmp is None else cmp.n_tokens_and_pad_rows)
        else:
            if cmp is not None:
                ops.linear_bf16(table_bf16, p.w_in, None, a_ids=_zero_ids(S, ids.device), res=p.in_rows, res_kind=1, res_mod=S, out=qkv[cap:])
            ops.linear_bf16(table_bf16, p.w_in, None, a_ids=a_ids, res=p.in_rows, res_kind=1, res_mod=S, out=qkv[:cap], c_ids=c_ids,
                            m_dev=None if cmp is None else cmp.n_live_tokens, n_alg=3 * E, k_alg=E)
        q, k, v = qkv[:, :W], qkv[:, W:2 * W], qkv[:, 2 * W:]
        if cmp is None:
            attn = ops.token_attention_bf16(q, k, v, n_seq, S, nhead, hd, scale, out_cols=EP)
        else:
            attn = ops.token_attention_rows_bf16(q, k, v, cmp.row_map, n_seq_dev, n_seq, S, nhead, hd, scale, out_cols=EP)
        sa = layer.self_attn
        pool = li == len(transformer.layers) - 1
        res = dict(res=table_bf16, res_kind=2, res_ids=res_ids) if li == 0 else dict(res=x, res_kind=3)
        ln2 = (layer.norm2.weight, layer.norm2.bias)
        if p.block:
            x = ops.encoder_block_bf16(attn, p.w0p, p.add_rows, (layer.norm1.weight, layer.norm1.bias), layer.norm1.eps, w1p=p.w1p, w2p=p.w2p,
                                       b2=layer.linear2.bias, ln2=ln2, ln2_eps=layer.norm2.eps, E=E, pool32=pool, **res, **rows)
            continue
        x1 = ops.linear_bf16(attn, p.w_o, p.b_o, res_pe=p.pe_p, res_period=S if li == 0 else 0, ln=p.ln1, ln_eps=layer.norm1.eps, ln_count=E,
                             n_alg=E, k_alg=E, **res, **rows)
        if p.ffn:
            x = ops.encoder_ffn_bf16(x1, p.w1p, p.w2p, layer.linear2.bias, ln2, layer.norm2.eps, E, pool32=pool, **rows)
            continue
        h = ops.linear_bf16(x1, p.w1, layer.linear1.bias, act='relu', k_alg=E, **rows)
        x = ops.linear_bf16(h, p.w2, p.b2, res=x1, res_kind=3, ln=p.ln2, ln_eps=layer.norm2.eps, ln_count=E, pool32=pool, n_alg=E, **rows)
    pooled = ops.mean_pool(x[:, :E], n_seq, S // 32, out=pooled_out if cmp is None else None, n_seq_dev=n_seq_dev)
    if cmp is not None:
        ops.gather_rows(cmp.seq_inv, pooled, pooled_out)
    return None


def encode_tokens_bf16(ids, table_bf16, pe, transformer, nhead, pooled_out):
    return _encode_layers_bf16(ids, None, table_bf16, pe, transformer, nhead, pooled_out)


def encode_tokens_bf16_compact(ids, table_bf16, pe, transformer, nhead, pooled_out, shared=None):
    if len(transformer.layers) != 1:
        raise NotImplementedError('the compacted bf16 path covers one encoder layer (compact_applicable_bf16)')
    return _encode_layers_bf16(ids, ops.compact_sequences(ids), table_bf16, pe, transformer, nhead, pooled_out, shared)


def compact_applicable_bf16(ids, transformer, nhead, E):
    M, S = ids.shape
    return (DEDUP and len(transformer.layers) == 1 and transformer.norm is None and E % nhead == 0 and E // nhead <= 32 and
            (E // nhead) % 2 == 0 and S in (32, 64, 128) and (M + 1) * S >= 4096 and ids.dtype == torch.int32 and ids.is_contiguous())


VOCAB_QKV = os.environ.get('LIME_VOCAB_QKV', '1') != '0'


def weight_state(sources, writes):
    return tuple((t.data_ptr(), tuple(t.shape), t._version) for t in sources), int(writes)


def weight_state_stale(recorded, current):
    if recorded is None:
        return 'never'
    (rec, rec_writes), (cur, cur_writes) = recorded, current
    if len(rec) != len(cur) or any(a[:2] != b[:2] for a, b in zip(rec, cur)):
        return 'moved'
    if any(a[2] != b[2] for a, b in zip(rec, cur)):
        return 'version'
    return 'writes' if rec_writes != cur_writes else None


def vocab_qkv_applicable(S, E, nhead):
    return S in (32, 64, 128) and E % nhead == 0 and E // nhead <= 32 and E % 4 == 0


_GENERATION = [0]


def _next_generation():
    _GENERATION[0] += 1
    return _GENERATION[0]


class WeightProducts:

    def __init__(self, budget):
        self.state = None
        self.budget = budget
        self.encoder = [{}, {}]
        self.generation = _next_generation()
        self.refreshes = 0

    def nbytes(self):
        return sum(t.numel() * t.element_size() for e in self.encoder for t in (e.get('ew'), e.get('pew')) if t is not None)

    def _buffer(self, old, shape, dtype, device):
        if old is not None and tuple(old.shape) == tuple(shape) and old.dtype == dtype and old.device == device:
            return old
        self.generation = _next_generation()
        return torch.empty(shape, dtype=dtype, device=device)

    def refresh(self, state, table, encoders, nhead, budget):
        self.budget = budget
        V, E = table.shape
        hd, W, dev = E // nhead, nhead * 32, table.device
        want = [vocab_qkv_applicable(S, E, nhead) for _, _, S in encoders]
        if sum(V * 3 * W * 4 for w in want if w) > budget:
            want = [False, False]
        with torch.no_grad():
            for ent, (pe, transformer, S), w in zip(self.encoder, encoders, want):
                if w:
                    sa = transformer.layers[0].self_attn
                    w_in = ops.pad_heads(sa.in_proj_weight, 3 * nhead, hd, 32)
                    b_in = ops.pad_heads(sa.in_proj_bias, 3 * nhead, hd, 32)
                    ent['ew'] = ops.linear(table, w_in, None, out=self._buffer(ent.get('ew'), (V, 3 * W), torch.float32, dev))
                    ent['pew'] = ops.linear(pe[:S], w_in, b_in, out=self._buffer(ent.get('pew'), (S, 3 * W), torch.float32, dev))
                elif 'ew' in ent:
                    del ent['ew'], ent['pew']
                    self.generation = _next_generation()
                packs = ent.get('ffn') or [None] * len(transformer.layers)
                for li, layer in enumerate(transformer.layers):
                    if not _ffn_sp_shape(layer, E):
                        packs[li] = None
                        continue
                    if packs[li] is None or packs[li][0].device != dev:
                        self.generation = _next_generation()
                        packs[li] = ops.ffn_pack_sp(layer.linear1.weight, layer.linear2.weight)
                    else:
                        ops.ffn_pack_sp(layer.linear1.weight, layer.linear2.weight, out=packs[li])
                ent['ffn'] = packs
                wops = ent.get('oproj') or [None] * len(transformer.layers)
                for li, layer in enumerate(transformer.layers):
                    if not (E <= 304 and E % 4 == 0):
                        wops[li] = None
                    elif wops[li] is None or wops[li].device != dev:
                        self.generation = _next_generation()
                        wops[li] = ops.oproj_pack_sp(layer.self_attn.out_proj.weight)
                    else:
                        ops.oproj_pack_sp(layer.self_attn.out_proj.weight, out=wops[li])
                ent['oproj'] = wops
        self.state = state
        self.refreshes += 1


class CROWN(NewsEncoder):

    def __init__(self, config):
        super().__init__(config)
        self.max_title_length = config.max_title_length
        self.max_body_length = config.max_abstract_length
        self.compute_dtype = getattr(config, 'compute_dtype', 'fp32')
        if self.compute_dtype not in ('fp32', 'bf16'):
            raise ValueError('compute_dtype must be fp32 or bf16')
        self.max_history_num = config.max_history_num
        self.category_embedding_dim = config.category_embedding_dim
        self.intent_embedding_dim = config.intent_embedding_dim
        self.category_embedding = nn.Embedding(config.category_num, config.category_embedding_dim)
        self.news_embedding_dim = config.intent_embedding_dim * 2 + config.category_embedding_dim + config.subCategory_embedding_dim
        self.head_num = config.head_num
        self.title_pos_encoder = PositionalEncoding(config.word_embedding_dim, config.dropout_rate, config.max_title_length)
        self.body_pos_encoder = PositionalEncoding(config.word_embedding_dim, config.dropout_rate, config.max_abstract_length)
        title_encoder_layers = TransformerEncoderLayer(config.word_embedding_dim, config.head_num, config.feedforward_dim,
                                                       config.dropout_rate, batch_first=True)
        self.title_transformer = TransformerEncoder(title_encoder_layers, config.num_layers)
        body_encoder_layers = TransformerEncoderLayer(config.word_embedding_dim, config.head_num, config.feedforward_dim,
                                                      config.dropout_rate, batch_first=True)
        self.body_transformer = TransformerEncoder(body_encoder_layers, config.num_layers)
        self.ISAB = ISAB(dim_in=config.word_embedding_dim, dim_out=config.word_embedding_dim, num_heads=config.isab_num_heads,
                         num_inds=config.isab_num_inds, ln=True)
        self.category_affine = nn.Linear(config.category_embedding_dim + config.subCategory_embedding_dim,
                                         config.category_embedding_dim)
        self.intent_num = config.intent_num
        self.alpha = config.alpha
        self.title_intent_attention = Attention(config.intent_embedding_dim, config.attention_dim)
        self.body_intent_attention = Attention(config.intent_embedding_dim, config.attention_dim)
        self.intent_layers = nn.ModuleList([nn.Linear(config.word_embedding_dim + config.category_embedding_dim,
                                                      config.intent_embedding_dim, bias=True) for _ in range(self.intent_num)])
        self.category_predictor = CategoryPredictor(config.intent_embedding_dim, config.category_num)

    def initialize(self):
        super().initialize()
        self.title_intent_attention.initialize()
        self.body_intent_attention.initialize()
        nn.init.xavier_uniform_(self.category_affine.weight)
        nn.init.zeros_(self.category_affine.bias)
        for intent_layer in self.intent_layers:
            nn.init.xavier_uniform_(intent_layer.weight)
            nn.init.zeros_(intent_layer.bias)
        nn.init.uniform_(self.category_embedding.weight, -0.1, 0.1)

    vocab_qkv_budget = 1 << 30

    def _product_sources(self):
        src = [self.word_embedding.weight]
        for pos, tr in ((self.title_pos_encoder, self.title_transformer), (self.body_pos_encoder, self.body_transformer)):
            sa = tr.layers[0].self_attn
            src += [sa.in_proj_weight, sa.in_proj_bias, pos.pe]
            for layer in tr.layers:
                src += [layer.linear1.weight, layer.linear2.weight, layer.self_attn.out_proj.weight]
        return src

    def weight_products(self, create=True):
        table = self.word_embedding.weight
        if not VOCAB_QKV or self.compute_dtype == 'bf16' or not table.is_cuda or not ops.split_gemm_on():
            return None
        wp = getattr(self, '_products', None)
        if wp is None and not create:
            return None
        state = weight_state(self._product_sources(), ops.PARAM_WRITES)
        budget = self.vocab_qkv_budget
        if wp is not None and weight_state_stale(wp.state, state) is None and wp.budget == budget:
            return wp
        if torch.cuda.is_current_stream_capturing():
            return None
        if wp is None:
            wp = self._products = WeightProducts(budget)
        wp.refresh(state, table, ((self.title_pos_encoder.table(), self.title_transformer, self.max_title_length),
                                  (self.body_pos_encoder.table(), self.body_transformer, self.max_body_length)), self.head_num, budget)
        return wp

    def products_key(self):
        used = self.weight_products(create=False) is not None
        wp = getattr(self, '_products', None)
        return (None if wp is None else wp.generation, used)

    def _apply(self, fn, *args, **kwargs):
        self._products = None
        return super()._apply(fn, *args, **kwargs)

    def _step_of(self, S, M, bf16):
        E = self.word_embedding_dim
        return min(max(1, MAX_TOKENS_PER_PASS // S),
                   max(1, (0x7FFFFFF0 // (3 * self.head_num * 32 * (2 if bf16 else 4))) // S - 2) if DEDUP else M,
                   max(1, (0x7FFFFFF0 // (((E + 7) // 8 * 8) * 2)) // S - 2) if bf16 else M)

    def _one_pass(self, title_text, content_text):
        M = title_text.shape[0]
        table = self.word_embedding.weight
        return (self.compute_dtype != 'bf16' and
                all(M <= self._step_of(ids.shape[1], M, False) and compact_applicable(ids, table, tr, self.head_num)
                    for ids, tr in ((title_text, self.title_transformer), (content_text, self.body_transformer))))

    def news_dedup_applicable(self, title_text, content_text):
        M = title_text.shape[0]
        return (DEDUP and title_text.is_cuda and self._one_pass(title_text, content_text) and 2 * (M + 1) < 4096 and
                self.intent_num * (M + 1) < 12288)

    def encode_flat(self, title_text, title_mask, content_text, category, subCategory, out, content_mask=None, news=None):
        _no_train_dropout(self, self.dropout_rate)
        M, T = title_text.shape
        L = content_text.shape[1]
        if T != self.max_title_length or L != self.max_body_length:
            raise ValueError('token tensors must be [*, %d] / [*, %d]' % (self.max_title_length, self.max_body_length))
        E, Dc, D = self.word_embedding_dim, self.category_embedding_dim, self.intent_embedding_dim
        k = self.intent_num
        dev = title_text.device
        table = self.word_embedding.weight
        kin = E + Dc
        ldx = (kin + 3) // 4 * 4
        dedup = news is not None
        if dedup:
            cmp_t, cmp_b, nw = news
            if not self.news_dedup_applicable(title_text, content_text) or nw.n != M or nw.count_mult != k:
                raise ValueError('news: the batch is outside news_dedup_applicable, or the lists are not this batch\'s (count_mult = intent_num)')
            category, subCategory = nw.cat_c, nw.sub_c
        R = M + 1 if dedup else M
        if out.shape[0] != R:
            raise ValueError('out must have %d rows' % R)
        xin = torch.empty((2 * R, ldx), dtype=torch.float32, device=dev)
        bf16 = self.compute_dtype == 'bf16'
        if bf16:
            table_b = ops.to_bf16(table, cols_out=(E + 7) // 8 * 8)
        main = torch.cuda.current_stream()
        side4 = _side_stream(dev, 4)
        side4.wait_stream(main)
        with torch.cuda.stream(side4):
            if dedup:
                side4.wait_event(nw.ready)
            sub_table = self.subCategory_embedding.weight
            ops.topic_rep(category, subCategory, self.category_embedding.weight, sub_table, self.category_affine.weight,
                          self.category_affine.bias, out=xin[:R, E:kin], emb_out=out[:, 2 * D:2 * D + Dc + sub_table.shape[1]])
            ops.topic_rep(category, subCategory, self.category_embedding.weight, sub_table, self.category_affine.weight,
                          self.category_affine.bias, out=xin[R:, E:kin])
            w_int = torch.nn.functional.pad(torch.cat([lin.weight for lin in self.intent_layers], dim=0), (0, ldx - kin))
            b_int = torch.cat([lin.bias for lin in self.intent_layers], dim=0)
            if ldx > kin:
                xin[:, kin:] = 0.0
        encoders = ((title_text, self.title_pos_encoder, self.title_transformer, T),
                    (content_text, self.body_pos_encoder, self.body_transformer, L))
        step_of = lambda S: self._step_of(S, M, bf16)
        one_pass = self._one_pass(title_text, content_text)
        compacted = not bf16 and (one_pass or any(compact_applicable(ids[m0:min(M, m0 + step_of(S))], table, tr, self.head_num)
                                                   for ids, _, tr, S in encoders for m0 in range(0, M, step_of(S))))
        wp = self.weight_products() if compacted else None
        prods = [None, None] if wp is None else wp.encoder
        if one_pass:
            (t_ids, t_pos, t_tr, _), (b_ids, b_pos, b_tr, _) = encoders
            side3 = _side_stream(dev, 3)
            side3.wait_stream(main)
            with torch.cuda.stream(side3):
                prep_t, prep_b = compact_prepare_many([(t_ids, t_pos.table(), t_tr), (b_ids, b_pos.table(), b_tr)], table, self.head_num,
                                                      cmps=(cmp_t, cmp_b) if dedup else None, products=prods)
            side1 = _side_stream(dev, 7)
            side1.wait_stream(side3)
            with torch.cuda.stream(side1):
                tb = compact_run(prep_t, table, t_pos.table(), t_tr, self.head_num, None if dedup else xin[:M, :E], dedup)
            main.wait_stream(side3)
            bb = compact_run(prep_b, table, b_pos.table(), b_tr, self.head_num, None if dedup else xin[M:, :E], dedup)
            main.wait_stream(side1)
            if dedup:
                ops.news_xin(tb, T // 32, bb, L // 32, nw, xin, E)
        else:
            side = _side_stream(dev, 7 if DEDUP else 1)
            side.wait_stream(main)
            for half, (ids, pos, tr, S) in enumerate(encoders):
                step = step_of(S)
                with torch.cuda.stream(side if half == 0 else main):
                    shared = {}
                    for m0 in range(0, M, step):
                        m1 = min(M, m0 + step)
                        if bf16:
                            if compact_applicable_bf16(ids[m0:m1], tr, self.head_num, E):
                                encode_tokens_bf16_compact(ids[m0:m1], table_b, pos.table(), tr, self.head_num,
                                                           xin[half * M + m0:half * M + m1, :E], shared=shared)
                            else:
                                encode_tokens_bf16(ids[m0:m1], table_b, pos.table(), tr, self.head_num, xin[half * M + m0:half * M + m1, :E])
                            continue
                        if compact_applicable(ids[m0:m1], table, tr, self.head_num):
                            encode_tokens_compact(ids[m0:m1], table, pos.table(), tr, self.head_num,
                                                  pooled_out=xin[half * M + m0:half * M + m1, :E], products=prods[half])
                            continue
                        encode_tokens(ids[m0:m1], table, pos.table(), tr, self.head_num,
                                      pooled_out=xin[half * M + m0:half * M + m1, :E])
            main.wait_stream(side)
        main.wait_stream(side4)
        if dedup:
            intents = torch.empty((2 * R, w_int.shape[0]), dtype=torch.float32, device=dev)
            ops.linear_group([dict(a=xin[half * R:(half + 1) * R], w=w_int, bias=b_int, act='relu', out=intents[half * R:(half + 1) * R],
                                   m_dev=nw.n_news) for half in range(2)])
        else:
            intents = ops.linear(xin, w_int, b_int, act='relu')
        A = self.title_intent_attention.affine1.out_features
        hidden = torch.empty((2 * R * k, A), dtype=torch.float32, device=dev)
        iv = intents.view(2 * R * k, D)
        rows_k = dict(m_dev=nw.n_news_mult) if dedup else {}
        ops.linear_group([dict(a=iv[half * R * k:(half + 1) * R * k], w=att.affine1.weight, bias=att.affine1.bias, act='tanh',
                               out=hidden[half * R * k:(half + 1) * R * k], **rows_k)
                          for half, att in enumerate((self.title_intent_attention, self.body_intent_attention))])
        ops.intent_fuse(iv, hidden, self.title_intent_attention.affine2.weight.view(-1),
                        self.body_intent_attention.affine2.weight.view(-1), out, R, k, D, A,
                        m_dev=nw.n_news if dedup else None)
        return out


class MHSA(NewsEncoder):

    def _encode(self, ids, mask, out, compact):
        n, T = ids.shape
        mha = self.multiheadAttention
        n_seq, rows, seqs, ids_r = n, {}, {}, ids.reshape(-1)
        if compact:
            if mask.dtype not in (torch.bool, torch.uint8):
                mask = mask.bool()
            mask = mask.contiguous()
            cmp = ops.compact_sequences(ops.mhsa_live_ids(ids, mask))
            mask = ops.mhsa_compact_mask(cmp, mask)
            n_seq, rows, seqs, ids_r = n + 1, dict(m_dev=cmp.n_rows), dict(n_seq_dev=cmp.n_compact), cmp.ids_c
        qkv = mha.project(table=self.word_embedding.weight, ids=ids_r, **rows)
        c = mha.attend(qkv, n_seq, T, mask, **seqs)
        hidden = ops.linear(c, self.attention.affine1.weight, self.attention.affine1.bias, act='tanh', **rows)
        pooled = ops.additive_pool(hidden, self.attention.affine2.weight.view(-1), c, n_seq, T, mask=mask, out=None if compact else out,
                                   **seqs)
        if compact:
            ops.gather_rows(cmp.seq_inv, pooled, out)

    def _compact_applicable(self, ids, n, T):
        mha = self.multiheadAttention
        return (DEDUP and (n + 1) * T >= 4096 and ids.dtype == torch.int32 and ids.is_contiguous() and mha.d_model % 4 == 0 and
                (3 * mha.h * mha.d_k) % 4 == 0 and mha.d_k <= 32 and mha.d_v <= 32 and T <= 512)

    def __init__(self, config):
        super().__init__(config)
        self.max_sentence_length = config.max_title_length
        self.feature_dim = config.head_num * config.head_dim
        self.multiheadAttention = MultiHeadAttention(config.head_num, config.word_embedding_dim, config.max_title_length,
                                                     config.max_title_length, config.head_dim, config.head_dim)
        self.attention = Attention(config.head_num * config.head_dim, config.attention_dim)
        self.news_embedding_dim = config.head_num * config.head_dim + config.category_embedding_dim + config.subCategory_embedding_dim
        self.category_embedding = nn.Embedding(config.category_num, config.category_embedding_dim)

    def initialize(self):
        super().initialize()
        self.multiheadAttention.initialize()
        self.attention.initialize()
        nn.init.uniform_(self.category_embedding.weight, -0.1, 0.1)

    def encode_flat(self, title_text, title_mask, content_text, category, subCategory, out, content_mask=None):
        _no_train_dropout(self, self.dropout_rate)
        M, T = title_text.shape
        F = self.feature_dim
        mask = title_mask.contiguous()
        step = max(1, MAX_TOKENS_PER_PASS // T)
        for m0 in range(0, M, step):
            m1 = min(M, m0 + step)
            ids = title_text[m0:m1]
            self._encode(ids, mask[m0:m1], out[m0:m1, :F], self._compact_applicable(ids, m1 - m0, T))
        ops.topic_rep(category, subCategory, self.category_embedding.weight, self.subCategory_embedding.weight,
                      emb_out=out[:, F:])
        return out


_ROW_COUNTS = {}


def _row_count(n, device):
    key = (device.type, device.index, n)
    t = _ROW_COUNTS.get(key)
    if t is None:
        t = _ROW_COUNTS[key] = torch.full((1,), n, dtype=torch.int32, device=device)
    return t


class CNN(NewsEncoder):

    def __init__(self, config):
        super().__init__(config)
        if getattr(config, 'compute_dtype', 'fp32') != 'fp32':
            raise NotImplementedError("compute_dtype %r: the CNN content encoder is built for fp32 (compute_dtype='fp32')" % config.compute_dtype)
        self.max_sentence_length = config.max_title_length
        self.cnn_kernel_num = config.cnn_kernel_num
        self.conv = Conv1D(config.cnn_method, config.word_embedding_dim, config.cnn_kernel_num, config.cnn_window_size)
        self.attention = Attention(config.cnn_kernel_num, config.attention_dim)
        self.news_embedding_dim = config.cnn_kernel_num + config.category_embedding_dim + config.subCategory_embedding_dim
        self.category_embedding = nn.Embedding(config.category_num, config.category_embedding_dim)
        nn.init.uniform_(self.category_embedding.weight, -0.1, 0.1)

    def initialize(self):
        super().initialize()
        self.attention.initialize()

    def _compact_applicable(self, ids):
        return (DEDUP and ids.dtype == torch.int32 and ids.is_contiguous() and self.cnn_kernel_num % 4 == 0 and
                self.attention.affine1.out_features % 4 == 0)

    def _encode(self, ids, mask, out, compact):
        n, T = ids.shape
        dev = ids.device
        K, A = self.cnn_kernel_num, self.attention.affine1.out_features
# ... 442 lines not shown
```

lime_cikm25_amd/ops.py:

```python
import ctypes
import math
import os

import torch

from . import _lib
from ._lib import LinearArgs, LIME_ACT, check


PROFILE = None


PARAM_WRITES = 0


def note_param_write():
    global PARAM_WRITES
    PARAM_WRITES += 1


def _stream():
    return ctypes.c_void_p(torch.cuda.current_stream().cuda_stream)


# ... 171 lines not shown
    _mat(table, 'table')
    rows, dim = ids.numel(), table.shape[1]
    if out is None:
        out = torch.empty((rows, dim), dtype=torch.float32, device=table.device)
    _mat(out, 'out')
    if pe is not None:
        _mat(pe, 'pe')
    check(lib.lime_embed_pe_f32(_p(ids), _p(table), _ld(table), _p(pe), _ld(pe) if pe is not None else 0, period, _p(out),
                                _ld(out), rows, dim, _stream()), 'lime_embed_pe_f32')
    return out


NOT_APPLICABLE = _lib.CONSTANTS['LIME_NOT_APPLICABLE']


def _token_attention_block(form, q=None, k=None, v=None, n_seq=0, S=0, n_head=0, head_dim=0, scale=1.0, key_mask=None, out=None,
                           head_stride=None, n_seq_dev=None, lse=None, row_map=None, qkv_vocab=None, pos_rows=None, ids=None, p=0.0,
                           seed=0, site=0):
    lib = _lib.load()
    a = _lib.TokenAttentionArgs()
    a.form = _lib.ATTN_FORM[form]
    hs = 32 if form in ('rows', 'vocab') else (head_dim if head_stride is None else head_stride)
    ptr = lambda t: None if t is None else t.data_ptr()
    mask = ws = None
    if form == 'vocab':
        _mat(qkv_vocab, 'qkv_vocab')
        _mat(pos_rows, 'pos_rows')
        W = n_head * 32
        if qkv_vocab.shape[1] != 3 * W or pos_rows.shape[1] != 3 * W or _ld(qkv_vocab) != _ld(pos_rows):
            raise ValueError('qkv_vocab and pos_rows must have 3 * n_head * 32 columns and one leading dimension')
        if pos_rows.shape[0] < S:
            raise ValueError('pos_rows must have at least S rows')
        _vec(ids, 'ids', dtype=torch.int32)
        if ids.numel() < n_seq * S:
            raise ValueError('ids must cover n_seq * S tokens')
        a.q, a.k, a.v = (qkv_vocab.data_ptr() + 4 * W * i for i in range(3))
        a.ld_qkv, a.pos_rows, a.row_map, device = _ld(qkv_vocab), ptr(pos_rows), ptr(ids), qkv_vocab.device
    else:
        for t, n in ((q, 'q'), (k, 'k'), (v, 'v')):
            _mat(t, n)
            if form == 'rows':
                if t.shape[1] != n_head * 32:
                    raise ValueError('%s must have n_head * 32 columns' % n)
            elif tuple(t.shape) != (n_seq * S, n_head * hs):
                raise ValueError('%s must be [n_seq * S, n_head * head_stride]' % n if form == 'dropout' else
                                 '%s must be [%d, %d]' % (n, n_seq * S, n_head * hs))
        if not (_ld(q) == _ld(k) == _ld(v)):
            raise ValueError('q, k, v must share one leading dimension' if form == 'dropout' else 'q, k and v must share one leading dimension')
        a.q, a.k, a.v, a.ld_qkv, device = ptr(q), ptr(k), ptr(v), _ld(q), q.device
    if form == 'rows':
        _vec(row_map, 'row_map', dtype=torch.int32)
        if row_map.numel() < n_seq * S:
            raise ValueError('row_map must cover n_seq * S tokens')
        a.row_map = ptr(row_map)
    if form in ('rows', 'vocab', 'count') and n_seq_dev is not None:
        a.n_seq_dev = ptr(_vec(n_seq_dev, 'n_seq_dev', 1, dtype=torch.int32))
    if out is None:
        out = torch.empty((n_seq * S, n_head * head_dim), dtype=torch.float32, device=device)
    _mat(out, 'out')
    if form == 'vocab' and (out.shape[0] != n_seq * S or out.shape[1] != n_head * head_dim):
        raise ValueError('out must be [n_seq * S, n_head * head_dim]')
    if form in ('plain', 'count', 'lse'):
        mask = _mask_u8(key_mask, 'key_mask')
        if mask is not None and mask.numel() != n_seq * S:
            raise ValueError('key_mask must have n_seq * S elements')
        if form == 'lse':
            if mask is not None or n_seq_dev is not None:
                raise ValueError('lse goes with the unmasked, host-counted call')
            a.lse = ptr(_vec(lse, 'lse', n_seq * S * n_head))
        a.key_mask = ptr(mask)
    if form == 'dropout':
        need = 0 if head_dim > 32 else lib.lime_token_attention_stats_workspace(n_seq, S, n_head)
        ws = _workspace(device, need) if need else None
        a.workspace, a.workspace_floats = ptr(ws), ws.numel() if ws is not None else 0
        a.dropout_p, a.dropout_seed, a.dropout_site = p, seed, site
    a.out, a.ldo = out.data_ptr(), _ld(out)
    a.n_seq, a.S, a.n_head, a.head_dim, a.head_stride, a.scale = n_seq, S, n_head, head_dim, hs, scale
    return a, out, (mask, ws)


def _token_attention(form, **kw):
    a, out, _keep = _token_attention_block(form, **kw)
    st = _lib.load().lime_token_attention_f32(ctypes.byref(a), _stream())
    if st == NOT_APPLICABLE:
        return None
    check(st, 'lime_token_attention_f32')
    return out


def token_attention(q, k, v, n_seq, S, n_head, head_dim, scale, key_mask=None, out=None, head_stride=None, n_seq_dev=None, lse=None):
    form = 'lse' if lse is not None else ('count' if n_seq_dev is not None else 'plain')
    return _token_attention(form, q=q, k=k, v=v, n_seq=n_seq, S=S, n_head=n_head, head_dim=head_dim, scale=scale, key_mask=key_mask,
                            out=out, head_stride=head_stride, n_seq_dev=n_seq_dev, lse=lse)


def token_attention_rows(q, k, v, row_map, n_seq_dev, n_seq, S, n_head, head_dim, scale, out=None):
    return _token_attention('rows', q=q, k=k, v=v, row_map=row_map, n_seq_dev=n_seq_dev, n_seq=n_seq, S=S, n_head=n_head,
                            head_dim=head_dim, scale=scale, out=out)


def token_attention_vocab(qkv_vocab, pos_rows, ids, n_seq_dev, n_seq, S, n_head, head_dim, scale, out=None):
    return _token_attention('vocab', qkv_vocab=qkv_vocab, pos_rows=pos_rows, ids=ids, n_seq_dev=n_seq_dev, n_seq=n_seq, S=S, n_head=n_head,
                            head_dim=head_dim, scale=scale, out=out)


def token_attention_plan(form, q=None, k=None, v=None, n_seq=0, S=0, n_head=0, head_dim=0, scale=1.0, key_mask=None, out=None,
                         head_stride=None, n_seq_dev=None, lse=None, row_map=None, qkv_vocab=None, pos_rows=None, ids=None, p=0.0, seed=0,
                         site=0):
    a, _out, _keep = _token_attention_block(form, q=q, k=k, v=v, n_seq=n_seq, S=S, n_head=n_head, head_dim=head_dim, scale=scale,
                                            key_mask=key_mask, out=out, head_stride=head_stride, n_seq_dev=n_seq_dev, lse=lse,
                                            row_map=row_map, qkv_vocab=qkv_vocab, pos_rows=pos_rows, ids=ids, p=p, seed=seed, site=site)
    plan = _lib.TokenAttentionPlan()
    st = _lib.load().lime_token_attention_plan_f32(ctypes.byref(a), ctypes.byref(plan))
    if st == NOT_APPLICABLE:
        return None
    check(st, 'lime_token_attention_plan_f32')
    return dict(family=_lib.ATTN_FAMILY[plan.family], stats_pass=_lib.ATTN_STATS[plan.stats_pass],
                kernels=[plan.name[i].value.decode() for i in range(plan.n_launches)])


class Compacted:
    __slots__ = ('n_seq', 'S', 'cap', 'seq_inv', 'seq_src', 'ids_c', 'row_map', 'tok_ids', 'tok_rows', 'counts')

    n_compact = property(lambda self: self.counts[0:1])
    n_rows = property(lambda self: self.counts[1:2])
    n_live_tokens = property(lambda self: self.counts[2:3])
    n_tokens_and_pad_rows = property(lambda self: self.counts[4:5])


def compact_sequences(ids, pad_base=None):
    lib = _lib.load()
    if ids.dim() != 2 or ids.dtype != torch.int32 or not ids.is_cuda or not ids.is_contiguous():
        raise TypeError('ids must be a contiguous CUDA int32 [n_seq, S] tensor')
    n_seq, S = ids.shape
    cap = (n_seq + 1) * S
    c = Compacted()
    c.n_seq, c.S, c.cap = n_seq, S, cap
    dev = ids.device
    buf = torch.empty(n_seq + 4 * cap + 8 + int(lib.lime_compact_sequences_workspace(n_seq)), dtype=torch.int32, device=dev)
    c.seq_inv = buf[:n_seq]
    o = n_seq
    c.ids_c, c.row_map, c.tok_ids, c.tok_rows = (buf[o + i * cap:o + (i + 1) * cap] for i in range(4))
    o += 4 * cap
    c.counts = buf[o:o + 5]
    work = buf[o + 8:]
    c.seq_src = work[n_seq:2 * n_seq + 1]
    check(lib.lime_compact_sequences(_p(ids), n_seq, S, cap if pad_base is None else pad_base, _p(c.seq_inv), _p(c.ids_c), _p(c.row_map),
                                     _p(c.tok_ids), _p(c.tok_rows), _p(c.counts), _p(work), _stream()), 'lime_compact_sequences')
    return c


class NewsCompacted:
    __slots__ = ('n', 'news_src', 'news_inv', 'title_row', 'body_row', 'cat_c', 'sub_c', 'fresh_c', 'life_c', 'counts', 'count_mult',
                 'ready')

    n_news = property(lambda self: self.counts[0:1])
    n_news_mult = property(lambda self: self.counts[1:2])


def _compacted_views(c, buf, n_seq, S):
    cap = (n_seq + 1) * S
    c.n_seq, c.S, c.cap = n_seq, S, cap
    c.seq_inv = buf[:n_seq]
    o = n_seq
    c.ids_c, c.row_map, c.tok_ids, c.tok_rows = (buf[o + i * cap:o + (i + 1) * cap] for i in range(4))
    o += 4 * cap
    c.counts = buf[o:o + 5]
    return o + 8


def compact_batch(title_ids, body_ids, cat, sub, fresh, life, count_mult=1):
    lib = _lib.load()
    for ids in (title_ids, body_ids):
        if ids.dim() != 2 or ids.dtype != torch.int32 or not ids.is_cuda or not ids.is_contiguous():
            raise TypeError('ids must be contiguous CUDA int32 [n, S] tensors')
    n, T = title_ids.shape
    L = body_ids.shape[1]
    if body_ids.shape[0] != n:
        raise ValueError('title_ids and body_ids must have one row per news')
    _vec(cat, 'cat', n, dtype=torch.int32)
    _vec(sub, 'sub', n, dtype=torch.int32)
    _vec(fresh, 'fresh', n)
    _vec(life, 'life', n)
    dev = title_ids.device
    words = lambda S: n + 4 * (n + 1) * S + 8
    buf = torch.empty(words(T) + words(L) + 8 * (n + 1) + 8 + int(lib.lime_compact_batch_workspace(n)), dtype=torch.int32, device=dev)
    t, b, w = Compacted(), Compacted(), NewsCompacted()
    o = _compacted_views(t, buf, n, T)
    o += _compacted_views(b, buf[o:], n, L)
    w.n, w.count_mult = n, count_mult
    w.news_src, w.title_row, w.body_row, w.cat_c, w.sub_c, fc, lc = (buf[o + i * (n + 1):o + (i + 1) * (n + 1)] for i in range(7))
    w.fresh_c, w.life_c = fc.view(torch.float32), lc.view(torch.float32)
    o += 7 * (n + 1)
    w.news_inv = buf[o:o + n]
    o += n + 1
    w.counts = buf[o:o + 4]
    work = buf[o + 8:]
    t.seq_src, b.seq_src = work[n:2 * n + 1], work[4 * n + 2:5 * n + 3]
    check(lib.lime_compact_batch(_p(title_ids), T, t.cap, _p(t.seq_inv), _p(t.ids_c), _p(t.row_map), _p(t.tok_ids), _p(t.tok_rows),
                                 _p(t.counts), _p(body_ids), L, b.cap, _p(b.seq_inv), _p(b.ids_c), _p(b.row_map), _p(b.tok_ids),
                                 _p(b.tok_rows), _p(b.counts), n, _p(cat), _p(sub), _p(fresh), _p(life), count_mult, _p(w.news_src),
                                 _p(w.news_inv), _p(w.title_row), _p(w.body_row), _p(w.cat_c), _p(w.sub_c), _p(w.fresh_c), _p(w.life_c),
                                 _p(w.counts), _p(work), _stream()), 'lime_compact_batch')
    w.ready = torch.cuda.Event()
    w.ready.record()
    return t, b, w


def news_xin(title_blocks, nblk_t, body_blocks, nblk_b, news, xin, dim):
    lib = _lib.load()
    _mat(title_blocks, 'title_blocks')
    _mat(body_blocks, 'body_blocks')
    _mat(xin, 'xin')
    cap = news.n + 1
    if title_blocks.shape != (cap * nblk_t, dim) or body_blocks.shape != (cap * nblk_b, dim):
        raise ValueError('title_blocks / body_blocks must be [(n + 1) * nblk, dim]')
    if xin.shape[0] != 2 * cap or xin.shape[1] < dim:
        raise ValueError('xin must be [2 (n + 1), >= dim]')
    check(lib.lime_news_xin_f32(_p(title_blocks), _ld(title_blocks), nblk_t, _p(body_blocks), _ld(body_blocks), nblk_b, _p(news.title_row),
                                _p(news.body_row), _p(news.n_news), _p(xin), _ld(xin), cap, dim, _stream()), 'lime_news_xin_f32')
    return xin


def pad_heads(src, n_blk, head_dim, head_stride):
    lib = _lib.load()
    vec = src.dim() == 1
    s2 = src.view(-1, 1) if vec else src
    _mat(s2, 'src')
    if s2.shape[0] != n_blk * head_dim:
        raise ValueError('src must have n_blk * head_dim rows')
    dst = torch.empty((n_blk * head_stride, s2.shape[1]), dtype=torch.float32, device=src.device)
    check(lib.lime_pad_heads_f32(_p(s2), _ld(s2), _p(dst), _ld(dst), n_blk, head_dim, head_stride, s2.shape[1], _stream()),
          'lime_pad_heads_f32')
    return dst.view(-1) if vec else dst


def mean_pool(x, n_seq, S, out=None, n_seq_dev=None):
    lib = _lib.load()
    _mat(x, 'x')
    if x.shape[0] != n_seq * S:
        raise ValueError('x must have n_seq * S rows')
    dim = x.shape[1]
    if out is None:
        out = torch.empty((n_seq, dim), dtype=torch.float32, device=x.device)
    _mat(out, 'out')
    if n_seq_dev is not None:
        _vec(n_seq_dev, 'n_seq_dev', dtype=torch.int32)
        check(lib.lime_mean_pool_count_f32(_p(x), _ld(x), _p(out), _ld(out), n_seq, S, dim, _p(n_seq_dev), _stream()),
              'lime_mean_pool_count_f32')
    else:
        check(lib.lime_mean_pool_f32(_p(x), _ld(x), _p(out), _ld(out), n_seq, S, dim, _stream()), 'lime_mean_pool_f32')
    return out


def bucketize(x, cuts=None):
    lib = _lib.load()
    x = _vec(x.contiguous(), 'x')
    out = torch.empty(x.shape, dtype=torch.int32, device=x.device)
    if cuts is not None:
        _vec(cuts, 'cuts')
        check(lib.lime_bucketize_cuts_f32(_p(x), _p(cuts), cuts.numel(), _p(out), x.numel(), _stream()), 'lime_bucketize_cuts_f32')
        return out
    check(lib.lime_bucketize_f32(_p(x), _p(out), x.numel(), _stream()), 'lime_bucketize_f32')
    return out


def mhsa_live_ids(ids, mask):
    lib = _lib.load()
    n, T = ids.shape
    m = _mask_u8(mask, 'mask')
    out = torch.empty_like(ids)
    check(lib.lime_mhsa_live_ids(_p(ids), _p(m), n, T, _p(out), _stream()), 'lime_mhsa_live_ids')
    return out


def mhsa_compact_mask(cmp, mask):
    lib = _lib.load()
    m = _mask_u8(mask, 'mask')
    mask_c = torch.empty((cmp.n_seq + 1, cmp.S), dtype=torch.uint8, device=cmp.ids_c.device)
    check(lib.lime_mhsa_compact_mask(_p(cmp.ids_c), _p(cmp.seq_src), _p(m), cmp.n_seq + 1, cmp.S, _p(mask_c), _stream()), 'lime_mhsa_compact_mask')
    return mask_c


def fuse_rows(a, b, gate=None, out=None):
    lib = _lib.load()
    _mat(a, 'a')
    _mat(b, 'b')
    if a.shape != b.shape or (gate is not None and gate.shape != a.shape):
        raise ValueError('a, b (and gate) must have one shape')
    if gate is not None:
        _mat(gate, 'gate')
    if out is None:
        out = torch.empty(tuple(a.shape), dtype=torch.float32, device=a.device)
    _mat(out, 'out')
    check(lib.lime_fuse_rows_f32(_p(a), _ld(a), _p(b), _ld(b), _p(gate), _ld(gate) if gate is not None else 0, _p(out), _ld(out),
                                 a.shape[0], a.shape[1], _stream()), 'lime_fuse_rows_f32')
    return out


def gather_rows(idx, table, out):
    lib = _lib.load()
    _vec(idx, 'idx', dtype=torch.int32)
    _mat(table, 'table')
    _mat(out, 'out')
    if out.shape[0] != idx.numel() or out.shape[1] != table.shape[1]:
        raise ValueError('out must be [len(idx), table.shape[1]]')
    check(lib.lime_gather_rows_f32(_p(idx), _p(table), _ld(table), _p(out), _ld(out), idx.numel(), table.shape[1], _stream()),
          'lime_gather_rows_f32')
    return out


FUSED_OCCURRENCE = os.environ.get('LIME_FUSED_OCCURRENCE', '0') == '1'
OCC_MODES = {'concat': _lib.CONSTANTS['LIME_OCC_CONCAT'], 'add': _lib.CONSTANTS['LIME_OCC_ADD'], 'gated': _lib.CONSTANTS['LIME_OCC_GATED']}


def cached_occurrence(mode, idx, freshness, lifetime, A, T, P=None, Q=None, cuts=None, out=None):
    lib = _lib.load()
    if mode not in OCC_MODES:
        raise ValueError('cached_occurrence: mode must be one of %s, got %r' % (sorted(OCC_MODES), mode))
    gated = mode == 'gated'
    if gated and (P is None or Q is None):
        raise ValueError("cached_occurrence: 'gated' needs P and Q")
    _mat(A, 'A')
    _mat(T, 'T')
    D = A.shape[1]
    R = _vec(idx, 'idx', dtype=torch.int32).numel()
    _vec(freshness, 'freshness', R)
    _vec(lifetime, 'lifetime', R)
    _vec(cuts, 'cuts')
    if T.shape[1] != D:
        raise ValueError('cached_occurrence: T has %d columns, A has %d' % (T.shape[1], D))
    if gated and (_mat(P, 'P').shape != A.shape or _mat(Q, 'Q').shape != T.shape):
        raise ValueError('cached_occurrence: P / Q must have the shapes of A / T')
    if out is None:
        out = torch.empty((R, D), dtype=torch.float32, device=A.device)
    if tuple(_mat(out, 'out').shape) != (R, D):
        raise ValueError('cached_occurrence: out must be [%d, %d], got %s' % (R, D, tuple(out.shape)))
    check(lib.lime_cached_occurrence_f32(OCC_MODES[mode], _p(idx), _p(freshness), _p(lifetime), _p(cuts), cuts.numel() if cuts is not None else 0,
                                         _p(A), _ld(A), _p(P) if gated else None, _ld(P) if gated else 0, _p(T), _ld(T),
                                         _p(Q) if gated else None, _ld(Q) if gated else 0, T.shape[0], _p(out), _ld(out), R, D, _stream()),
          'lime_cached_occurrence_f32')
    return out


def topic_rep(cat, sub, cat_table, sub_table, w=None, bias=None, out=None, emb_out=None):
    lib = _lib.load()
    _vec(cat, 'cat', dtype=torch.int32)
    _vec(sub, 'sub', cat.numel(), dtype=torch.int32)
    _mat(cat_table, 'cat_table')
    _mat(sub_table, 'sub_table')
    if not (cat_table.is_contiguous() and sub_table.is_contiguous()):
        raise ValueError('embedding tables must be contiguous')
    rows, dc, ds = cat.numel(), cat_table.shape[1], sub_table.shape[1]
    dout = 0
    if w is not None:
        _mat(w, 'w')
        if not w.is_contiguous() or w.shape[1] != dc + ds:
            raise ValueError('w must be contiguous [dout, dc + ds]')
        dout = w.shape[0]
        if out is None:
            out = torch.empty((rows, dout), dtype=torch.float32, device=cat.device)
        _mat(out, 'out')
        if tuple(out.shape) != (rows, dout):
            raise ValueError('out must be [rows, dout]')
        _vec(bias, 'bias', dout)
    if emb_out is not None:
        _mat(emb_out, 'emb_out')
        if tuple(emb_out.shape) != (rows, dc + ds):
            raise ValueError('emb_out must be [rows, dc + ds]')
    check(lib.lime_topic_rep_f32(_p(cat), _p(sub), _p(cat_table), _p(sub_table), dc, ds, _p(w), _p(bias), dout,
                                 _p(out) if w is not None else None, _ld(out) if w is not None else 0, _p(emb_out),
                                 _ld(emb_out) if emb_out is not None else 0, rows, _stream()), 'lime_topic_rep_f32')
    return out


def intent_fuse(intents, att_hidden, affine2_t, affine2_b, content, M, k, D, A, m_dev=None):
    lib = _lib.load()
    _mat(intents, 'intents')
    _mat(att_hidden, 'att_hidden')
    if not (intents.is_contiguous() and att_hidden.is_contiguous()):
        raise ValueError('intents / att_hidden must be contiguous')
    if tuple(intents.shape) != (2 * M * k, D) or tuple(att_hidden.shape) != (2 * M * k, A):
        raise ValueError('intents / att_hidden have the wrong shape')
    _mat(content, 'content')
    if content.shape[0] != M or content.shape[1] < 2 * D:
        raise ValueError('content must be [M, >= 2D]')
    if m_dev is not None:
        check(lib.lime_intent_fuse_count_f32(_p(intents), _p(att_hidden), _p(_vec(affine2_t, 'affine2_t', A)),
                                             _p(_vec(affine2_b, 'affine2_b', A)), _p(content), _ld(content), M, k, D, A,
                                             _p(_vec(m_dev, 'm_dev', 1, dtype=torch.int32)), _stream()), 'lime_intent_fuse_count_f32')
        return content
    check(lib.lime_intent_fuse_f32(_p(intents), _p(att_hidden), _p(_vec(affine2_t, 'affine2_t', A)),
                                   _p(_vec(affine2_b, 'affine2_b', A)), _p(content), _ld(content), M, k, D, A, _stream()),
          'lime_intent_fuse_f32')
    return content


def additive_pool(hidden, affine2, x, n_seq, S, mask=None, out=None, n_seq_dev=None):
    lib = _lib.load()
    _mat(hidden, 'hidden')
    _mat(x, 'x')
    A, D = hidden.shape[1], x.shape[1]
    if hidden.shape[0] != n_seq * S or x.shape[0] != n_seq * S:
        raise ValueError('hidden and x must have n_seq * S rows')
    if out is None:
        out = torch.empty((n_seq, D), dtype=torch.float32, device=x.device)
    _mat(out, 'out')
    m = _mask_u8(mask, 'mask')
    if n_seq_dev is not None:
        _vec(n_seq_dev, 'n_seq_dev', 1, dtype=torch.int32)
    check(lib.lime_additive_pool_count_f32(_p(hidden), _ld(hidden), _p(_vec(affine2, 'affine2', A)), A, _p(x), _ld(x), D, _p(m),
                                           _p(n_seq_dev), _p(out), _ld(out), n_seq, S, _stream()), 'lime_additive_pool_f32')
    return out


def fill_pad_rows(ids, src, dst, S):
    lib = _lib.load()
    _vec(ids, 'ids', dtype=torch.int32)
    _mat(src, 'src')
    _mat(dst, 'dst')
    if dst.shape[0] != ids.numel() or src.shape[0] < S or src.shape[1] != dst.shape[1]:
        raise ValueError('fill_pad_rows: dst must be [len(ids), cols], src [>= S, cols]')
    check(lib.lime_fill_pad_rows_f32(_p(ids), _p(src), _ld(src), _p(dst), _ld(dst), ids.numel(), S, dst.shape[1], _stream()),
          'lime_fill_pad_rows_f32')
    return dst


def additive_pool_bwd(hidden, affine2, x, dout, n_seq, S, mask=None):
    lib = _lib.load()
    _mat(hidden, 'hidden')
    _mat(x, 'x')
    _mat(dout, 'dout')
    A, D = hidden.shape[1], x.shape[1]
    if hidden.shape[0] != n_seq * S or x.shape[0] != n_seq * S or tuple(dout.shape) != (n_seq, D):
        raise ValueError('hidden and x must have n_seq * S rows, dout must be [n_seq, D]')
    dh = torch.empty((n_seq * S, A), dtype=torch.float32, device=x.device)
    dx = torch.empty((n_seq * S, D), dtype=torch.float32, device=x.device)
    part = torch.empty((max(n_seq, 1), A), dtype=torch.float32, device=x.device)
    m = _mask_u8(mask, 'mask')
    check(lib.lime_additive_pool_bwd_f32(_p(hidden), _ld(hidden), _p(_vec(affine2, 'affine2', A)), A, _p(x), _ld(x), D, _p(m), _p(dout),
                                         _ld(dout), _p(dh), _ld(dh), _p(dx), _ld(dx), _p(part), n_seq, S, _stream()), 'lime_additive_pool_bwd_f32')
    da2 = colsum(part[:n_seq]) if n_seq else torch.zeros(A, dtype=torch.float32, device=x.device)
    return dh, da2, dx


CAND_ATTN_BY_HEAD = True


def cand_attn_weights(qp, kp, mask, B, N, H, D, n_head, hist_div=1):
    lib = _lib.load()
    if B % hist_div:
        raise ValueError('B must be a multiple of hist_div')
    Bh = B // hist_div
    _vec(qp, 'qp', B * N * D)
    _vec(kp, 'kp', Bh * H * D)
    m = _mask_u8(mask, 'mask')
    if m.numel() != Bh * H:
        raise ValueError('mask must be [B / hist_div, H]')
    agg = torch.empty((B, H), dtype=torch.float32, device=qp.device)
    by_head = (N + H) * (D // n_head + 1) * 4 <= 64 * 1024
    if hist_div > 1 and not (CAND_ATTN_BY_HEAD and by_head):
        kp, m, hist_div = kp.view(Bh, H * D).repeat_interleave(hist_div, dim=0).view(-1), m.view(Bh, H).repeat_interleave(hist_div, dim=0), 1
    if CAND_ATTN_BY_HEAD and by_head:
        n_ws = int(lib.lime_cand_attn_weights_workspace(B, N, H, n_head))
        ws = torch.empty(max(n_ws, 1), dtype=torch.float32, device=qp.device)
        check(lib.lime_cand_attn_weights_shared_f32(_p(qp), _p(kp), _p(m), _p(agg), B, N, H, D, n_head, hist_div, _p(ws), n_ws, _stream()),
              'lime_cand_attn_weights_shared_f32')
        return agg
    check(lib.lime_cand_attn_weights_f32(_p(qp), _p(kp), _p(m), _p(agg), B, N, H, D, n_head, _stream()),
          'lime_cand_attn_weights_f32')
    return agg


def gate_ln_sage(y, x, scale, bias, gamma, beta, eps, groups, H, D, row_div, n_src, node_const=None):
    lib = _lib.load()
    src_rows = (groups // row_div) * H * D
    x = _vec(x.contiguous(), 'x', src_rows)
    y = _vec(y.contiguous(), 'y', src_rows)
    scale = _vec(scale.contiguous(), 'scale', groups * H)
    out = torch.empty((groups * H, D), dtype=torch.float32, device=x.device)
    mean = torch.empty((groups, D), dtype=torch.float32, device=x.device)
    nc = _vec(node_const.contiguous(), 'node_const', D) if node_const is not None else None
    check(lib.lime_gate_ln_sage_f32(_p(y), _p(x), _p(scale), _p(_vec(bias, 'bias', D)), _p(_vec(gamma, 'gamma', D)), _p(_vec(beta, 'beta', D)),
                                    eps, _p(out), _p(nc) if nc is not None else None, _p(mean), groups, H, D, row_div, n_src, _stream()),
          'lime_gate_ln_sage_f32')
    return out, mean


def gate_ln(y, x, scale, bias, gamma, beta, eps=1e-5):
    lib = _lib.load()
    D = x.shape[-1]
    x = _vec(x.contiguous(), 'x')
    y = _vec(y.contiguous(), 'y', x.numel())
    rows = x.numel() // D
    out = torch.empty_like(x)
    check(lib.lime_gate_ln_f32(_p(y), _p(x), _p(_vec(scale.contiguous(), 'scale', rows)), _p(_vec(bias, 'bias', D)),
                               _p(_vec(gamma, 'gamma', D)), _p(_vec(beta, 'beta', D)), eps, _p(out), rows, D, _stream()),
          'lime_gate_ln_f32')
    return out


def sage_mean(hist, user_nodes, B, H, n_src, D):
    lib = _lib.load()
    _vec(hist, 'hist', B * H * D)
    _vec(user_nodes, 'user_nodes')
    n_user = user_nodes.numel() // D
    out = torch.empty((B, D), dtype=torch.float32, device=hist.device)
    check(lib.lime_sage_mean_f32(_p(hist), _p(user_nodes), _p(out), B, H, n_user, n_src, D, _stream()), 'lime_sage_mean_f32')
    return out


def interest_match(kp, qp, g, cand, remaining, B, N, H, A, D, scale, alpha, beta, use_weight, use_penalty, want_logits=True,
                   want_user=True):
    lib = _lib.load()
    _vec(kp, 'kp', B * H * A)
    _vec(qp, 'qp', B * N * A)
    _vec(g, 'g', B * H * D)
    _vec(cand, 'cand', B * N * D)
    if want_logits and use_weight:
        remaining = _vec(remaining.contiguous(), 'remaining', B * N)
    user = torch.empty((B, N, D), dtype=torch.float32, device=kp.device) if want_user else None
    logits = torch.empty((B, N), dtype=torch.float32, device=kp.device) if want_logits else None
    check(lib.lime_interest_match_f32(_p(kp), _p(qp), _p(g), _p(cand), _p(remaining) if want_logits and use_weight else None,
                                      _p(user), _p(logits), B, N, H, A, D, scale, alpha, beta, int(use_weight),
                                      int(use_penalty), _stream()), 'lime_interest_match_f32')
    return user, logits
# ... 1935 lines not shown
```

Before: 27120.

## Fuse news key bucketing and topic rep, wave-level scan, cache intent weights

Reworks the single-block batch scan to keep rows in registers and use wave shuffles instead of a shared-memory Hillis-Steele scan with many barriers. Adds a fused news_keys kernel that computes the bucket pair, both topic-rep outputs and padding zeroing in one launch. Caches the concatenated intent-layer weights in the weight-products cache and widens the graph invalidation key to cover them. Together these aim to cut launch count, per-call weight concatenation and barrier overhead, at the cost of more cache-staleness logic.

Measured after the change: 27950, median of 6. +3.0%, better.

```diff
diff --git a/include/lime_hip.h b/include/lime_hip.h
--- a/include/lime_hip.h
+++ b/include/lime_hip.h
@@ -273,6 +273,11 @@
 int lime_topic_rep_f32(const int32_t* cat, const int32_t* sub, const float* cat_table, const float* sub_table,
                        int32_t dc, int32_t ds, const float* w, const float* bias, int32_t dout, float* out, int64_t ldo,
                        float* emb_out, int64_t ld_emb, int64_t rows, void* stream);
+
+int lime_news_keys_f32(const int32_t* cat, const int32_t* sub, const float* fresh, const float* life, const float* cuts, int32_t n_cuts,
+                       int32_t nb, const float* cat_table, const float* sub_table, int32_t dc, int32_t ds, const float* w,
+                       const float* bias, int32_t dout, float* xin, int64_t ldx, int32_t col0, float* emb_out, int64_t ld_emb,
+                       int32_t* pair, int64_t rows, void* stream);
 
 int lime_intent_fuse_f32(const float* intents, const float* att_hidden, const float* affine2_t, const float* affine2_b,
                          float* content, int64_t ldc, int64_t M, int32_t k, int32_t D, int32_t A, void* stream);
diff --git a/lime_cikm25_amd/csrc/compact.hip b/lime_cikm25_amd/csrc/compact.hip
--- a/lime_cikm25_amd/csrc/compact.hip
+++ b/lime_cikm25_amd/csrc/compact.hip
@@ -124,20 +124,19 @@
     else count_seq(b.ids, w - n, b.S, b.live_cnt);
 }
 
-__device__ __forceinline__ void scan_side_write(const SeqSide& d, int n, int lo, int hi, int ps, int pt, int n_live, int n_tok) {
+__device__ __forceinline__ void scan_side_put(const SeqSide& d, int s, int c, int& ps, int& pt, int n_live) {
+    if (c > 0) {
+        d.seq_src[ps] = s;
+        d.seq_inv[s] = ps;
+        d.tok_off[ps] = pt;
+        ++ps;
+        pt += c;
+    } else {
+        d.seq_inv[s] = n_live;
+    }
+}
+__device__ __forceinline__ void scan_side_tail(const SeqSide& d, int n, int n_live, int n_tok) {
     const int tid = threadIdx.x;
-    for (int s = lo; s < hi; ++s) {
-        const int c = d.live_cnt[s];
-        if (c > 0) {
-            d.seq_src[ps] = s;
-            d.seq_inv[s] = ps;
-            d.tok_off[ps] = pt;
-            ++ps;
-            pt += c;
-        } else {
-            d.seq_inv[s] = n_live;
-        }
-    }
     for (int i = n_live + 1 + tid; i <= n; i += 1024) d.seq_src[i] = -1;
     if (tid == 0) {
         d.seq_src[n_live] = -1;
@@ -150,62 +149,97 @@
     }
 }
 
+struct NewsRow { int ct, cb, cat, sub, fresh, life; };
+__device__ __forceinline__ NewsRow load_row(const SeqSide& t, const SeqSide& b, const NewsSide& w, int s) {
+    return {t.live_cnt[s], b.live_cnt[s], w.cat[s], w.sub[s], w.fresh[s], w.life[s]};
+}
+
+template <int PER>
 __global__ __launch_bounds__(1024) void batch_scan_kernel(const SeqSide t, const SeqSide b, const NewsSide w, int n) {
-    __shared__ int part[5][1024];
-    const int tid = threadIdx.x;
+    __shared__ int wave_first[16];
+    __shared__ int wave_tot[5][16];
+    const int tid = threadIdx.x, lane = tid & 63, wave = tid >> 6;
     const int per = (n + 1023) / 1024;
     const int lo = min(n, tid * per), hi = min(n, lo + per);
+    NewsRow reg[PER > 0 ? PER : 1];
+    if (PER > 0) {
+#pragma unroll
+        for (int i = 0; i < PER; ++i) reg[i] = load_row(t, b, w, min(lo + i, n - 1));
+    }
+    auto each_own = [&](auto&& f) {
+        if constexpr (PER > 0) {
+#pragma unroll
+            for (int i = 0; i < PER; ++i) {
+                if (lo + i < hi) f(lo + i, reg[i]);
+            }
+        } else {
+            for (int s = lo; s < hi; ++s) f(s, load_row(t, b, w, s));
+        }
+    };
     int first = 0x7FFFFFFF;
-    for (int s = hi - 1; s >= lo; --s)
-        if (t.live_cnt[s] == 0 && b.live_cnt[s] == 0) first = s;
-    part[0][tid] = first;
+    int v[5] = {0, 0, 0, 0, 0};
+    each_own([&](int s, const NewsRow& r) {
+        v[0] += r.ct > 0; v[1] += r.ct;
+        v[2] += r.cb > 0; v[3] += r.cb;
+        if (r.ct == 0 && r.cb == 0) first = min(first, s);
+    });
+#pragma unroll
+    for (int o = 32; o > 0; o >>= 1) first = min(first, __shfl_xor(first, o));
+    if (lane == 0) wave_first[wave] = first;
     __syncthreads();
-    for (int o = 512; o > 0; o >>= 1) {
-        if (tid < o) part[0][tid] = min(part[0][tid], part[0][tid + o]);
-        __syncthreads();
-    }
-    first = part[0][0];
+    first = wave_first[lane & 15];
+#pragma unroll
+    for (int o = 8; o > 0; o >>= 1) first = min(first, __shfl_xor(first, o));
+    const bool has_pad = first != 0x7FFFFFFF;
+    NewsRow key = {0, 0, 0, 0, 0, 0};
+    if (has_pad) key = load_row(t, b, w, first);
+    auto repeats = [&](const NewsRow& r) {
+        return has_pad & (r.ct == 0) & (r.cb == 0) & (r.cat == key.cat) & (r.sub == key.sub) & (r.fresh == key.fresh) & (r.life == key.life);
+    };
+    each_own([&](int, const NewsRow& r) { v[4] += !repeats(r); });
+    int inc[5];
+#pragma unroll
+    for (int i = 0; i < 5; ++i) inc[i] = v[i];
+#pragma unroll
+    for (int o = 1; o < 64; o <<= 1) {
+#pragma unroll
+        for (int i = 0; i < 5; ++i) {
+            const int up = __shfl_up(inc[i], o);
+            if (lane >= o) inc[i] += up;
+        }
+    }
+    if (lane == 63) {
+#pragma unroll
+        for (int i = 0; i < 5; ++i) wave_tot[i][wave] = inc[i];
+    }
     __syncthreads();
-    const bool has_pad = first != 0x7FFFFFFF;
-    int kc = 0, ks = 0, kf = 0, kl = 0;
-    if (has_pad) { kc = w.cat[first]; ks = w.sub[first]; kf = w.fresh[first]; kl = w.life[first]; }
-    auto repeats = [&](int s) {
-        return has_pad && t.live_cnt[s] == 0 && b.live_cnt[s] == 0 && w.cat[s] == kc && w.sub[s] == ks && w.fresh[s] == kf && w.life[s] == kl;
-    };
-    int v[5] = {0, 0, 0, 0, 0};
-    for (int s = lo; s < hi; ++s) {
-        const int ct = t.live_cnt[s], cb = b.live_cnt[s];
-        v[0] += ct > 0; v[1] += ct;
-        v[2] += cb > 0; v[3] += cb;
-        v[4] += !repeats(s);
-    }
-#pragma unroll
-    for (int i = 0; i < 5; ++i) part[i][tid] = v[i];
-    __syncthreads();
-    for (int o = 1; o < 1024; o <<= 1) {
-        int a[5] = {0, 0, 0, 0, 0};
-        if (tid >= o) {
-#pragma unroll
-            for (int i = 0; i < 5; ++i) a[i] = part[i][tid - o];
-        }
-        __syncthreads();
-#pragma unroll
-        for (int i = 0; i < 5; ++i) part[i][tid] += a[i];
-        __syncthreads();
-    }
-    scan_side_write(t, n, lo, hi, part[0][tid] - v[0], part[1][tid] - v[1], part[0][1023], part[1][1023]);
-    scan_side_write(b, n, lo, hi, part[2][tid] - v[2], part[3][tid] - v[3], part[2][1023], part[3][1023]);
-    const int n_live = part[4][1023];
-    int pn = part[4][tid] - v[4];
-    for (int s = lo; s < hi; ++s) {
-        if (repeats(s)) {
+    int ex[5], tot[5];
+#pragma unroll
+    for (int i = 0; i < 5; ++i) {
+        int x = lane < 16 ? wave_tot[i][lane] : 0;
+#pragma unroll
+        for (int o = 1; o < 16; o <<= 1) {
+            const int up = __shfl_up(x, o);
+            if (lane >= o) x += up;
+        }
+        const int before = __shfl(x, wave > 0 ? wave - 1 : 0);
+        tot[i] = __shfl(x, 15);
+        ex[i] = (wave > 0 ? before : 0) + inc[i] - v[i];
+    }
+    const int n_live = tot[4];
+    each_own([&](int s, const NewsRow& r) {
+        scan_side_put(t, s, r.ct, ex[0], ex[1], tot[0]);
+        scan_side_put(b, s, r.cb, ex[2], ex[3], tot[2]);
+        if (repeats(r)) {
             w.news_inv[s] = n_live;
         } else {
-            w.news_src[pn] = s;
-            w.news_inv[s] = pn;
-            ++pn;
-        }
-    }
+            w.news_src[ex[4]] = s;
+            w.news_inv[s] = ex[4];
+            ++ex[4];
+        }
+    });
+    scan_side_tail(t, n, tot[0], tot[1]);
+    scan_side_tail(b, n, tot[2], tot[3]);
     for (int i = n_live + 1 + tid; i <= n; i += 1024) w.news_src[i] = -1;
     if (tid == 0) {
         const int n_news = n_live + (has_pad ? 1 : 0);
@@ -285,7 +319,8 @@
                         (int*)fresh_c, (int*)life_c, news_counts, count_mult};
     const int seq_blocks = (n + 1 + 3) / 4;
     hipLaunchKernelGGL(batch_count_kernel, dim3((unsigned)((2L * n + 3) / 4)), dim3(256), 0, s, t, b, n);
-    hipLaunchKernelGGL(batch_scan_kernel, dim3(1), dim3(1024), 0, s, t, b, w, n);
+    if ((n + 1023) / 1024 <= 2) hipLaunchKernelGGL(batch_scan_kernel<2>, dim3(1), dim3(1024), 0, s, t, b, w, n);
+    else hipLaunchKernelGGL(batch_scan_kernel<0>, dim3(1), dim3(1024), 0, s, t, b, w, n);
     hipLaunchKernelGGL(batch_emit_kernel, dim3((unsigned)(2 * seq_blocks + (n + 1 + 255) / 256)), dim3(256), 0, s, t, b, w, n, seq_blocks);
     return lime_check_launch("lime_compact_batch");
 }
diff --git a/lime_cikm25_amd/csrc/news_tail_f32.hip b/lime_cikm25_amd/csrc/news_tail_f32.hip
--- a/lime_cikm25_amd/csrc/news_tail_f32.hip
+++ b/lime_cikm25_amd/csrc/news_tail_f32.hip
@@ -1,14 +1,13 @@
 #include "common.h"
+#include "dev_helpers.h"
 
 namespace {
 
-__global__ __launch_bounds__(64) void topic_rep_kernel(const int* __restrict__ cat, const int* __restrict__ sub,
-                                                        const float* __restrict__ cat_table, const float* __restrict__ sub_table,
-                                                        int dc, int ds, const float* __restrict__ w, const float* __restrict__ bias,
-                                                        int dout, float* __restrict__ out, long ldo, float* __restrict__ emb_out,
-                                                        long ld_emb) {
-    __shared__ float e[256];
-    const long r = blockIdx.x;
+__device__ __forceinline__ void topic_rep_row(long r, const int* __restrict__ cat, const int* __restrict__ sub,
+                                              const float* __restrict__ cat_table, const float* __restrict__ sub_table, int dc, int ds,
+                                              const float* __restrict__ w, const float* __restrict__ bias, int dout,
+                                              float* __restrict__ out, float* __restrict__ out2, long ldo, float* __restrict__ emb_out,
+                                              long ld_emb, float* e) {
     const int din = dc + ds;
     const float* crow = cat_table + (long)cat[r] * dc;
     const float* srow = sub_table + (long)sub[r] * ds;
@@ -23,9 +22,39 @@
             const float* wr = w + (long)o * din;
             float acc = 0.f;
             for (int i = 0; i < din; ++i) acc += wr[i] * e[i];
-            out[r * ldo + o] = acc + (bias ? bias[o] : 0.f);
-        }
-    }
+            const float y = acc + (bias ? bias[o] : 0.f);
+            out[r * ldo + o] = y;
+            if (out2) out2[r * ldo + o] = y;
+        }
+    }
+}
+
+__global__ __launch_bounds__(64) void topic_rep_kernel(const int* __restrict__ cat, const int* __restrict__ sub,
+                                                        const float* __restrict__ cat_table, const float* __restrict__ sub_table,
+                                                        int dc, int ds, const float* __restrict__ w, const float* __restrict__ bias,
+                                                        int dout, float* __restrict__ out, long ldo, float* __restrict__ emb_out,
+                                                        long ld_emb) {
+    __shared__ float e[256];
+    topic_rep_row(blockIdx.x, cat, sub, cat_table, sub_table, dc, ds, w, bias, dout, out, nullptr, ldo, emb_out, ld_emb, e);
+}
+
+__global__ __launch_bounds__(64) void news_keys_kernel(const int* __restrict__ cat, const int* __restrict__ sub,
+                                                        const float* __restrict__ fresh, const float* __restrict__ life,
+                                                        const float* __restrict__ cuts, int n_cuts, int nb,
+                                                        const float* __restrict__ cat_table, const float* __restrict__ sub_table,
+                                                        int dc, int ds, const float* __restrict__ w, const float* __restrict__ bias,
+                                                        int dout, float* __restrict__ xin, long ldx, int col0, long rows,
+                                                        float* __restrict__ emb_out, long ld_emb, int* __restrict__ pair) {
+    __shared__ float e[256];
+    const long j = blockIdx.x;
+    if (threadIdx.x == 0) pair[j] = lime_dev::bucket_of(fresh[j], cuts, n_cuts) * nb + lime_dev::bucket_of(life[j], cuts, n_cuts);
+    float* top = xin + col0;
+    float* bot = xin + rows * ldx + col0;
+    for (int c = dout + threadIdx.x; c < (int)ldx - col0; c += 64) {
+        top[j * ldx + c] = 0.f;
+        bot[j * ldx + c] = 0.f;
+    }
+    topic_rep_row(j, cat, sub, cat_table, sub_table, dc, ds, w, bias, dout, top, bot, ldx, emb_out, ld_emb, e);
 }
 
 }
@@ -42,6 +71,24 @@
     hipLaunchKernelGGL(topic_rep_kernel, dim3((unsigned)rows), dim3(64), 0, (hipStream_t)stream, cat, sub, cat_table, sub_table, dc,
                        ds, w, bias, dout, out, (long)ldo, emb_out, (long)ld_emb);
     return lime_check_launch("lime_topic_rep_f32");
+}
+
+extern "C" int lime_news_keys_f32(const int32_t* cat, const int32_t* sub, const float* fresh, const float* life, const float* cuts,
+                                  int32_t n_cuts, int32_t nb, const float* cat_table, const float* sub_table, int32_t dc, int32_t ds,
+                                  const float* w, const float* bias, int32_t dout, float* xin, int64_t ldx, int32_t col0, float* emb_out,
+                                  int64_t ld_emb, int32_t* pair, int64_t rows, void* stream) {
+    LIME_REQUIRE(cat && sub && fresh && life && cat_table && sub_table && w && xin && emb_out && pair, LIME_ERR_BAD_ARG,
+                 "lime_news_keys_f32: NULL pointer");
+    LIME_REQUIRE(cuts ? (n_cuts >= 0 && n_cuts <= 4096 && nb == n_cuts + 1) : nb == 10, LIME_ERR_BAD_ARG,
+                 "lime_news_keys_f32: nb %d does not match the cut points (%d given; 10 buckets built in)", nb, cuts ? n_cuts : 9);
+    LIME_REQUIRE(dc > 0 && ds > 0 && dc + ds <= 256, LIME_ERR_UNSUPPORTED, "lime_news_keys_f32: dc + ds must be in (0, 256]");
+    LIME_REQUIRE(dout > 0 && col0 >= 0 && ldx >= (int64_t)col0 + dout && ldx < 0x7FFFFFFFL && ld_emb >= dc + ds, LIME_ERR_BAD_ARG,
+                 "lime_news_keys_f32: bad dims dout=%d col0=%d ldx=%ld ld_emb=%ld", dout, col0, (long)ldx, (long)ld_emb);
+    if (rows <= 0) return rows == 0 ? LIME_OK : LIME_ERR_BAD_ARG;
+    LIME_REQUIRE(rows < 0x7FFFFFFFL, LIME_ERR_UNSUPPORTED, "lime_news_keys_f32: too many rows");
+    hipLaunchKernelGGL(news_keys_kernel, dim3((unsigned)rows), dim3(64), 0, (hipStream_t)stream, cat, sub, fresh, life, cuts, n_cuts, nb,
+                       cat_table, sub_table, dc, ds, w, bias, dout, xin, (long)ldx, col0, (long)rows, emb_out, (long)ld_emb, pair);
+    return lime_check_launch("lime_news_keys_f32");
 }
 
 namespace {
diff --git a/lime_cikm25_amd/model.py b/lime_cikm25_amd/model.py
--- a/lime_cikm25_amd/model.py
+++ b/lime_cikm25_amd/model.py
@@ -100,13 +100,21 @@
     def weights_changed(self):
         ops.note_param_write()
 
+    def _kept_key(self):
+        ne = self._modules['news_encoder']
+        found = self.__dict__.get('_kept_key_fns')
+        enc = ne if self.plain else ne._modules['base_news_encoder']
+        if found is None or found[0] is not ne or found[1] is not enc:
+            found = self.__dict__['_kept_key_fns'] = (ne, enc, tuple(getattr(m, name) for m, name in ((enc, 'products_key'), (ne, 'tables_key'))
+                                                                      if hasattr(m, name)))
+        keys = tuple(fn() for fn in found[2])
+        return keys or None
+
     def _sync_weight_products(self):
-        enc = self.content_encoder
-        if hasattr(enc, 'products_key'):
-            key = enc.products_key()
-            if key != getattr(self, '_products_key', None):
-                self._products_key = key
-                self._graphs = {}
+        key = self._kept_key()
+        if key != getattr(self, '_products_key', None):
+            self._products_key = key
+            self._graphs = {}
 
     def initialize(self):
         self.news_encoder.initialize()
@@ -160,9 +168,7 @@
                 out = self._forward_impl(*static)
             entry = (graph, [static[i] for i in _USED], out)
             self._graphs[key] = entry
-            enc = self.content_encoder
-            if hasattr(enc, 'products_key'):
-                self._products_key = enc.products_key()
+            self._products_key = self._kept_key()
         graph, static_used, out = entry
         keep = ops.multi_copy(list(zip(static_used, used)))
         graph.replay()
diff --git a/lime_cikm25_amd/newsEncoders.py b/lime_cikm25_amd/newsEncoders.py
--- a/lime_cikm25_amd/newsEncoders.py
+++ b/lime_cikm25_amd/newsEncoders.py
@@ -256,15 +256,18 @@
                 news = ops.compact_batch(title_text, content_text, category, subCategory, freshness.contiguous(), lifetime.contiguous(),
                                          count_mult=enc.intent_num)
             nw = news[2]
-            side.wait_stream(main)
-            with torch.cuda.stream(side):
-                side.wait_event(nw.ready)
-                pair = torch.add(fe.buckets(nw.life_c), fe.buckets(nw.fresh_c), alpha=nb)
-                table, _ = self.occurrence_tables()
+            table = self._kept_tables()
+            forked = table is None
+            if forked:
+                side.wait_stream(main)
+                with torch.cuda.stream(side):
+                    table = self._compute_occurrence_tables()
             content = torch.empty((M + 1, cdim), dtype=torch.float32, device=dev)
-            enc.encode_flat(title_text, title_mask, content_text, category, subCategory, content, news=news)
-            main.wait_stream(side)
-            rep_c = ops.linear(content, self.project.weight[:, :cdim], None, res=table, res_ids=pair, m_dev=nw.n_news)
+            enc.encode_flat(title_text, title_mask, content_text, category, subCategory, content, news=news,
+                            buckets=(nb, fe.cuts_on(dev)))
+            if forked:
+                main.wait_stream(side)
+            rep_c = ops.linear(content, self.project.weight[:, :cdim], None, res=table[0], res_ids=nw.pair, m_dev=nw.n_news)
             return ops.gather_rows(nw.news_inv, rep_c, torch.empty((M, rep_c.shape[1]), dtype=torch.float32, device=dev))
         side.wait_stream(main)
         with torch.cuda.stream(side):
@@ -277,6 +280,47 @@
         return ops.linear(content, self.project.weight[:, :cdim], None, res=table, res_ids=pair)
 
     def occurrence_tables(self):
+        kept = self._kept_tables()
+        return kept if kept is not None else self._compute_occurrence_tables()
+
+    def _table_sources(self):
+        fe = self.freshness_encoder
+        src = [fe.freshness_embedding.weight, fe.lifetime_embedding.weight, fe.dense.weight, fe.dense.bias]
+        if self.fusion_method == 'gated':
+            src += [self.gate.weight, self.gate.bias]
+        elif self.fusion_method == 'concat' and not isinstance(self.project, nn.Identity):
+            src += [self.project.weight, self.project.bias]
+        return src
+
+    def _kept_tables(self):
+        src = kept_sources(self, '_table_paths', self._table_sources, self.fusion_method)
+        if not WEIGHT_PREP_CACHE or not src[0].is_cuda or (torch.is_grad_enabled() and any(t.requires_grad for t in src)):
+            return None
+        kept = getattr(self, '_tables', None)
+        state = weight_state(src, ops.PARAM_WRITES)
+        if kept is not None and weight_state_stale(kept.state, state) is None:
+            return kept.T, kept.Q
+        if torch.cuda.is_current_stream_capturing():
+            return None
+        if kept is None:
+            kept = self._tables = OccurrenceTables()
+        with torch.no_grad():
+            kept.refresh(state, *self._compute_occurrence_tables())
+        return kept.T, kept.Q
+
+    def tables_key(self):
+        if self.fusion_method != 'concat' or isinstance(self.project, nn.Identity):
+            return None
+        kept = getattr(self, '_tables', None)
+        used = kept is not None and self._kept_tables() is not None
+        return (None if kept is None else kept.generation, used)
+
+    def _apply(self, fn, *args, **kwargs):
+        self.__dict__['_table_paths'] = None
+        self._tables = None
+        return super()._apply(fn, *args, **kwargs)
+
+    def _compute_occurrence_tables(self):
         fe = self.freshness_encoder
         E, nb = fe.freshness_embedding.embedding_dim, fe.num_buckets
         cdim = self.base_news_encoder.news_embedding_dim
@@ -842,6 +886,7 @@
 
 
 VOCAB_QKV = os.environ.get('LIME_VOCAB_QKV', '1') != '0'
+WEIGHT_PREP_CACHE = os.environ.get('LIME_WEIGHT_PREP_CACHE', '1') != '0'
 
 
 def weight_state(sources, writes):
@@ -851,6 +896,8 @@
 def weight_state_stale(recorded, current):
     if recorded is None:
         return 'never'
+    if recorded == current:
+        return None
     (rec, rec_writes), (cur, cur_writes) = recorded, current
     if len(rec) != len(cur) or any(a[:2] != b[:2] for a, b in zip(rec, cur)):
         return 'moved'
@@ -859,6 +906,52 @@
     return 'writes' if rec_writes != cur_writes else None
 
 
+class SourcePaths:
+
+    def __init__(self, links, leaves, tag):
+        self.links, self.leaves, self.tag = links, leaves, tag
+
+    @classmethod
+    def find(cls, root, tensors, tag=None):
+        where = {}
+        for prefix, mod in root.named_modules(remove_duplicate=False):
+            for d in (mod._parameters, mod._buffers):
+                for name, t in d.items():
+                    if t is not None:
+                        where.setdefault(id(t), (prefix, d, name))
+        links, leaves, seen = [], [], set()
+        for t in tensors:
+            if id(t) not in where:
+                return None
+            prefix, d, name = where[id(t)]
+            leaves.append((d, name))
+            mod, path = root, ''
+            for hop in (prefix.split('.') if prefix else []):
+                child = mod._modules[hop]
+                path += '.' + hop
+                if path not in seen:
+                    seen.add(path)
+                    links.append((mod._modules, hop, child))
+                mod = child
+        return cls(links, leaves, tag)
+
+    def tensors(self, tag=None):
+        if tag != self.tag or any(d.get(name) is not child for d, name, child in self.links):
+            return None
+        return [d[name] for d, name in self.leaves]
+
+
+def kept_sources(module, slot, slow, tag=None):
+    paths = module.__dict__.get(slot)
+    if paths is not None:
+        ts = paths.tensors(tag)
+        if ts is not None:
+            return ts
+    ts = slow()
+    module.__dict__[slot] = SourcePaths.find(module, ts, tag)
+    return ts
+
+
 def vocab_qkv_applicable(S, E, nhead):
     return S in (32, 64, 128) and E % nhead == 0 and E // nhead <= 32 and E % 4 == 0
 
@@ -877,6 +970,7 @@
         self.state = None
         self.budget = budget
         self.encoder = [{}, {}]
+        self.intent = {}
         self.generation = _next_generation()
         self.refreshes = 0
 
@@ -889,7 +983,7 @@
         self.generation = _next_generation()
         return torch.empty(shape, dtype=dtype, device=device)
 
-    def refresh(self, state, table, encoders, nhead, budget):
+    def refresh(self, state, table, encoders, nhead, budget, intent_layers=None, ldx=0):
         self.budget = budget
         V, E = table.shape
         hd, W, dev = E // nhead, nhead * 32, table.device
@@ -897,6 +991,20 @@
         if sum(V * 3 * W * 4 for w in want if w) > budget:
             want = [False, False]
         with torch.no_grad():
+            if intent_layers is not None:
+                D, kin = intent_layers[0].weight.shape
+                k = len(intent_layers)
+                fresh_w = self.intent.get('w') is None or tuple(self.intent['w'].shape) != (k * D, ldx) or self.intent['w'].device != dev
+                w = self.intent['w'] = self._buffer(self.intent.get('w'), (k * D, ldx), torch.float32, dev)
+                b = self.intent['b'] = self._buffer(self.intent.get('b'), (k * D,), torch.float32, dev)
+                if fresh_w and ldx > kin:
+                    w[:, kin:].zero_()
+                for i, lin in enumerate(intent_layers):
+                    w[i * D:(i + 1) * D, :kin].copy_(lin.weight)
+                    b[i * D:(i + 1) * D].copy_(lin.bias)
+            elif self.intent:
+                self.intent = {}
+                self.generation = _next_generation()
             for ent, (pe, transformer, S), w in zip(self.encoder, encoders, want):
                 if w:
                     sa = transformer.layers[0].self_attn
@@ -932,6 +1040,28 @@
         self.refreshes += 1
 
 
+class OccurrenceTables:
+
+    def __init__(self):
+        self.state = None
+        self.T = self.Q = None
+        self.generation = _next_generation()
+        self.refreshes = 0
+
+    def _into(self, old, new):
+        if new is None:
+            return None
+        if old is None or old.shape != new.shape or old.dtype != new.dtype or old.device != new.device:
+            self.generation = _next_generation()
+            old = torch.empty_like(new, memory_format=torch.contiguous_format)
+        return old.copy_(new)
+
+    def refresh(self, state, T, Q):
+        self.T, self.Q = self._into(self.T, T), self._into(self.Q, Q)
+        self.state = state
+        self.refreshes += 1
+
+
 class CROWN(NewsEncoder):
 
     def __init__(self, config):
@@ -987,6 +1117,8 @@
             src += [sa.in_proj_weight, sa.in_proj_bias, pos.pe]
             for layer in tr.layers:
                 src += [layer.linear1.weight, layer.linear2.weight, layer.self_attn.out_proj.weight]
+        for lin in self.intent_layers:
+            src += [lin.weight, lin.bias]
         return src
 
     def weight_products(self, create=True):
@@ -996,16 +1128,18 @@
         wp = getattr(self, '_products', None)
         if wp is None and not create:
             return None
-        state = weight_state(self._product_sources(), ops.PARAM_WRITES)
+        state = weight_state(kept_sources(self, '_product_paths', self._product_sources), ops.PARAM_WRITES)
         budget = self.vocab_qkv_budget
-        if wp is not None and weight_state_stale(wp.state, state) is None and wp.budget == budget:
+        if wp is not None and weight_state_stale(wp.state, state) is None and wp.budget == budget and bool(wp.intent) == WEIGHT_PREP_CACHE:
             return wp
         if torch.cuda.is_current_stream_capturing():
             return None
         if wp is None:
             wp = self._products = WeightProducts(budget)
+        kin = self.word_embedding_dim + self.category_embedding_dim
         wp.refresh(state, table, ((self.title_pos_encoder.table(), self.title_transformer, self.max_title_length),
-                                  (self.body_pos_encoder.table(), self.body_transformer, self.max_body_length)), self.head_num, budget)
+                                  (self.body_pos_encoder.table(), self.body_transformer, self.max_body_length)), self.head_num, budget,
+                   intent_layers=list(self.intent_layers) if WEIGHT_PREP_CACHE else None, ldx=(kin + 3) // 4 * 4)
         return wp
 
     def products_key(self):
@@ -1014,6 +1148,7 @@
         return (None if wp is None else wp.generation, used)
 
     def _apply(self, fn, *args, **kwargs):
+        self.__dict__['_product_paths'] = None
         self._products = None
         return super()._apply(fn, *args, **kwargs)
 
@@ -1035,7 +1170,8 @@
         return (DEDUP and title_text.is_cuda and self._one_pass(title_text, content_text) and 2 * (M + 1) < 4096 and
                 self.intent_num * (M + 1) < 12288)
 
-    def encode_flat(self, title_text, title_mask, content_text, category, subCategory, out, content_mask=None, news=None):
+    def encode_flat(self, title_text, title_mask, content_text, category, subCategory, out, content_mask=None, news=None,
+                    buckets=None):
         _no_train_dropout(self, self.dropout_rate)
         M, T = title_text.shape
         L = content_text.shape[1]
@@ -1061,20 +1197,6 @@
         if bf16:
             table_b = ops.to_bf16(table, cols_out=(E + 7) // 8 * 8)
         main = torch.cuda.current_stream()
-        side4 = _side_stream(dev, 4)
-        side4.wait_stream(main)
-        with torch.cuda.stream(side4):
-            if dedup:
-                side4.wait_event(nw.ready)
-            sub_table = self.subCategory_embedding.weight
-            ops.topic_rep(category, subCategory, self.category_embedding.weight, sub_table, self.category_affine.weight,
-                          self.category_affine.bias, out=xin[:R, E:kin], emb_out=out[:, 2 * D:2 * D + Dc + sub_table.shape[1]])
-            ops.topic_rep(category, subCategory, self.category_embedding.weight, sub_table, self.category_affine.weight,
-                          self.category_affine.bias, out=xin[R:, E:kin])
-            w_int = torch.nn.functional.pad(torch.cat([lin.weight for lin in self.intent_layers], dim=0), (0, ldx - kin))
-            b_int = torch.cat([lin.bias for lin in self.intent_layers], dim=0)
-            if ldx > kin:
-                xin[:, kin:] = 0.0
         encoders = ((title_text, self.title_pos_encoder, self.title_transformer, T),
                     (content_text, self.body_pos_encoder, self.body_transformer, L))
         step_of = lambda S: self._step_of(S, M, bf16)
@@ -1083,6 +1205,28 @@
                                                    for ids, _, tr, S in encoders for m0 in range(0, M, step_of(S))))
         wp = self.weight_products() if compacted else None
         prods = [None, None] if wp is None else wp.encoder
+        side4 = _side_stream(dev, 4)
+        side4.wait_stream(main)
+        with torch.cuda.stream(side4):
+            if dedup:
+                side4.wait_event(nw.ready)
+            sub_table = self.subCategory_embedding.weight
+            emb_out = out[:, 2 * D:2 * D + Dc + sub_table.shape[1]]
+            if dedup and buckets is not None:
+                nw.pair = ops.news_keys(nw, buckets[0], buckets[1], self.category_embedding.weight, sub_table, self.category_affine.weight,
+                                        self.category_affine.bias, xin, E, emb_out)
+            else:
+                ops.topic_rep(category, subCategory, self.category_embedding.weight, sub_table, self.category_affine.weight,
+                              self.category_affine.bias, out=xin[:R, E:kin], emb_out=emb_out)
+                ops.topic_rep(category, subCategory, self.category_embedding.weight, sub_table, self.category_affine.weight,
+                              self.category_affine.bias, out=xin[R:, E:kin])
+                if ldx > kin:
+                    xin[:, kin:] = 0.0
+            if wp is not None and wp.intent:
+                w_int, b_int = wp.intent['w'], wp.intent['b']
+            else:
+                w_int = torch.nn.functional.pad(torch.cat([lin.weight for lin in self.intent_layers], dim=0), (0, ldx - kin))
+                b_int = torch.cat([lin.bias for lin in self.intent_layers], dim=0)
         if one_pass:
             (t_ids, t_pos, t_tr, _), (b_ids, b_pos, b_tr, _) = encoders
             side3 = _side_stream(dev, 3)
diff --git a/lime_cikm25_amd/ops.py b/lime_cikm25_amd/ops.py
--- a/lime_cikm25_amd/ops.py
+++ b/lime_cikm25_amd/ops.py
@@ -347,7 +347,8 @@
 
 class NewsCompacted:
     __slots__ = ('n', 'news_src', 'news_inv', 'title_row', 'body_row', 'cat_c', 'sub_c', 'fresh_c', 'life_c', 'counts', 'count_mult',
-                 'ready')
+                 'ready',
+                 'pair')
 
     n_news = property(lambda self: self.counts[0:1])
     n_news_mult = property(lambda self: self.counts[1:2])
@@ -567,6 +568,35 @@
                                  _p(out) if w is not None else None, _ld(out) if w is not None else 0, _p(emb_out),
                                  _ld(emb_out) if emb_out is not None else 0, rows, _stream()), 'lime_topic_rep_f32')
     return out
+
+
+def news_keys(news, nb, cuts, cat_table, sub_table, w, bias, xin, col0, emb_out):
+    lib = _lib.load()
+    rows = news.n + 1
+    _mat(cat_table, 'cat_table')
+    _mat(sub_table, 'sub_table')
+    _mat(w, 'w')
+    if not (cat_table.is_contiguous() and sub_table.is_contiguous()):
+        raise ValueError('embedding tables must be contiguous')
+    dc, ds = cat_table.shape[1], sub_table.shape[1]
+    if not w.is_contiguous() or w.shape[1] != dc + ds:
+        raise ValueError('w must be contiguous [dout, dc + ds]')
+    dout = w.shape[0]
+    _vec(bias, 'bias', dout)
+    _vec(cuts, 'cuts')
+    if cuts.numel() + 1 != nb if cuts is not None else nb != 10:
+        raise ValueError('news_keys: %d buckets need %d cut points (None: the 10 buckets built in)' % (nb, nb - 1))
+    _mat(xin, 'xin')
+    if xin.shape[0] != 2 * rows or col0 < 0 or xin.shape[1] < col0 + dout or not xin.is_contiguous():
+        raise ValueError('xin must be contiguous [2 (n + 1), >= col0 + dout]')
+    _mat(emb_out, 'emb_out')
+    if tuple(emb_out.shape) != (rows, dc + ds):
+        raise ValueError('emb_out must be [n + 1, dc + ds]')
+    pair = torch.empty((rows,), dtype=torch.int32, device=xin.device)
+    check(lib.lime_news_keys_f32(_p(news.cat_c), _p(news.sub_c), _p(news.fresh_c), _p(news.life_c), _p(cuts),
+                                 cuts.numel() if cuts is not None else 0, nb, _p(cat_table), _p(sub_table), dc, ds, _p(w), _p(bias), dout,
+                                 _p(xin), xin.shape[1], col0, _p(emb_out), _ld(emb_out), _p(pair), rows, _stream()), 'lime_news_keys_f32')
+    return pair
 
 
 def intent_fuse(intents, att_hidden, affine2_t, affine2_b, content, M, k, D, A, m_dev=None):
```
